# jsign/go-curdleproofs

Hardware: NVIDIA B200
Metric: whisk_shuffle_proof_roundtrips_per_s (GenerateWhiskShuffleProof + IsValidWhiskShuffleProof, n=128) (higher is better)
Workload: dtype u32 (12x32-bit Montgomery limbs, IMAD.WIDE)

## Files before the change

go-curdleproofs_b200/binding.py:

```python
from __future__ import annotations

import ctypes as C
import os
import re

HERE = os.path.dirname(os.path.abspath(__file__))
HEADER = os.path.join(HERE, "..", "include", "curdle_b200.h")

FP_BYTES = 48
FR_BYTES = 32
G1_AFFINE_BYTES = 96
G1_JAC_BYTES = 144


class CdlError(RuntimeError):
    def __init__(self, code: int, msg: str):
        super().__init__(f"curdle_b200 error {code}: {msg}")
        self.code = code
        self.msg = msg


def lib_path() -> str:
    return os.environ.get("CDL_LIB") or os.path.join(HERE, "libcurdle_b200.so")


def declared_symbols():
    txt = open(HEADER).read()
    txt = re.sub(r"/\*.*?\*/", "", txt, flags=re.S)
    return sorted(set(re.findall(r"\b(cdl_[a-z0-9_]+)\s*\(", txt)))


_LIB = None


def load_library():
    global _LIB
    if _LIB is not None:
        return _LIB
    p = lib_path()
    if not os.path.exists(p):
        raise RuntimeError(
            f"{p} is missing: build it with `python -c 'import __graft_entry__ as g; g.build()'` "
            "(nvcc, sm_100a).  There is no CPU fallback.")
    lib = C.CDLL(p)
    vp, sz, i32, u32p = C.c_void_p, C.c_size_t, C.c_int32, C.POINTER(C.c_uint32)
    lib.cdl_abi_version.restype = C.c_uint32
    lib.cdl_create.argtypes = [C.c_int, C.POINTER(vp)]
    lib.cdl_destroy.argtypes = [vp]
    lib.cdl_destroy.restype = None
    lib.cdl_last_error.argtypes = [vp]
    lib.cdl_last_error.restype = C.c_char_p
    lib.cdl_device_info.argtypes = [vp, C.POINTER(i32), C.POINTER(i32), C.c_char_p, sz]
    lib.cdl_g1_msm.argtypes = [vp, vp, vp, sz, vp]
    lib.cdl_g1_msm_batch.argtypes = [vp, vp, vp, u32p, sz, vp]
    lib.cdl_g1_msm_batch_device.argtypes = [vp, vp, vp, vp, vp, sz, vp, vp, vp]
    lib.cdl_g1_scalar_mul_affine.argtypes = [vp, vp, vp, sz, sz, vp]
    lib.cdl_g1_fold.argtypes = [vp, vp, vp, vp, sz]
    lib.cdl_g1_batch_to_affine.argtypes = [vp, vp, sz, vp]
    lib.cdl_g1_sum_affine.argtypes = [vp, vp, sz, vp]
    lib.cdl_g1_compress.argtypes = [vp, vp, sz, vp]
    lib.cdl_g1_decompress.argtypes = [vp, vp, sz, vp, vp]
    lib.cdl_fp_mul.argtypes = [vp, vp, vp, sz, vp]
    lib.cdl_int_peak.argtypes = [vp, C.c_int, C.c_int, C.POINTER(C.c_double), C.POINTER(C.c_double)]
    lib.cdl_int_peak_cfg.argtypes = [vp, C.c_int, C.c_int, C.c_int, C.c_int, C.POINTER(C.c_double), C.POINTER(C.c_double)]
    u64, i32p = C.c_uint64, C.POINTER(C.c_int32)
    lib.cdl_rand_new.argtypes = [u64, C.POINTER(vp)]
    lib.cdl_rand_free.argtypes = [vp]
    lib.cdl_rand_free.restype = None
    lib.cdl_rand_get_frs.argtypes = [vp, sz, vp]
    lib.cdl_rand_get_g1_affines.argtypes = [vp, vp, sz, vp]
    lib.cdl_rand_generate_permutation.argtypes = [vp, sz, u32p]
    lib.cdl_crs_generate.argtypes = [vp, sz, vp, C.POINTER(vp)]
    lib.cdl_crs_from_points.argtypes = [vp, sz, vp, C.POINTER(vp)]
    lib.cdl_crs_export.argtypes = [vp, vp, vp]
    lib.cdl_crs_ell.argtypes = [vp]
    lib.cdl_crs_ell.restype = sz
    lib.cdl_crs_free.argtypes = [vp]
    lib.cdl_crs_free.restype = None
    lib.cdl_shuffle_permute_commit.argtypes = [vp, vp, vp, vp, u32p, vp, vp, vp, vp, vp, vp]
    lib.cdl_prove.argtypes = [vp, vp, vp, vp, vp, vp, vp, u32p, vp, vp, vp, vp, sz, C.POINTER(sz)]
    lib.cdl_verify.argtypes = [vp, vp, vp, sz, vp, vp, vp, vp, vp, vp, i32p]
    lib.cdl_whisk_generate_shuffle_proof.argtypes = [vp, vp, vp, vp, vp, vp, sz]
    lib.cdl_whisk_is_valid_shuffle_proof.argtypes = [vp, vp, vp, vp, sz, sz, vp, sz, vp, i32p]
    lib.cdl_whisk_generate_shuffle_proof_batch.argtypes = [vp, vp, sz, vp, C.POINTER(vp), vp, vp, sz, i32p]
    lib.cdl_whisk_is_valid_shuffle_proof_batch.argtypes = [vp, vp, sz, vp, vp, vp, sz, C.POINTER(vp), i32p, i32p]
    lib.cdl_whisk_generate_tracker_proof_batch.argtypes = [vp, sz, vp, vp, C.POINTER(vp), vp, i32p]
    lib.cdl_whisk_is_valid_tracker_proof_batch.argtypes = [vp, sz, vp, vp, vp, i32p, i32p]
    lib.cdl_whisk_match_trackers.argtypes = [vp, sz, vp, sz, vp, i32p, i32p]
    lib.cdl_host_selftest.argtypes = [vp, vp, vp, vp]
    lib.cdl_host_selftest_fibers.argtypes = [C.c_uint32, C.c_uint32, vp, C.POINTER(C.c_int32)]
    lib.cdl_engine_stats.argtypes = [vp, vp, vp, vp, vp, C.c_int]
    lib.cdl_engine_busy_ms.argtypes = [vp, C.POINTER(C.c_double)]
    lib.cdl_set_lanes.argtypes = [vp, i32]
    lib.cdl_launch_count.argtypes = [vp]
    lib.cdl_launch_count.restype = u64
    f32p = C.POINTER(C.c_float)
    lib.cdl_dev_alloc.argtypes = [vp, sz, C.POINTER(vp)]
    lib.cdl_dev_free.argtypes = [vp, vp]
    lib.cdl_dev_upload.argtypes = [vp, vp, vp, sz]
    lib.cdl_dev_download.argtypes = [vp, vp, vp, sz]
    lib.cdl_g1_scalar_mul_affine_device.argtypes = [vp, vp, vp, sz, sz, vp]
    lib.cdl_g1_fold_device.argtypes = [vp, vp, vp, vp, sz]
    lib.cdl_g1_msm_device.argtypes = [vp, vp, vp, sz, C.c_uint32, C.c_uint32, i32, vp, f32p]
    lib.cdl_set_msm_window.argtypes = [vp, i32]
    lib.cdl_set_msm_batch_affine.argtypes = [vp, i32]
    lib.cdl_set_fixed_base_min_batch.argtypes = [vp, i32]
    lib.cdl_comm_unique_id.argtypes = [vp]
    lib.cdl_comm_init.argtypes = [vp, vp, i32, i32]
    lib.cdl_comm_destroy.argtypes = [vp]
    lib.cdl_comm_partition.argtypes = [sz, i32, i32, i32, i32p, i32p, i32p, i32p]
    lib.cdl_comm_partition.restype = None
    lib.cdl_g1_msm_sharded_device.argtypes = [vp, vp, vp, sz, vp, f32p]
    lib.cdl_g1_msm_sharded.argtypes = [vp, vp, vp, sz, vp]
    no_status = ("cdl_comm_partition", "cdl_destroy", "cdl_last_error", "cdl_abi_version", "cdl_rand_free", "cdl_crs_free", "cdl_crs_ell",
                 "cdl_launch_count")
    for name in declared_symbols():
        fn = getattr(lib, name)
        if name not in no_status:
            fn.restype = i32
    _LIB = lib
    return lib


class Context:

    def __init__(self, device: int = 0):
        self.lib = load_library()
        h = C.c_void_p()
        rc = self.lib.cdl_create(device, C.byref(h))
        if rc != 0:
            raise CdlError(rc, "cdl_create failed (no CUDA device? this library has no CPU fallback)")
        self.h = h

    def close(self):
        if getattr(self, "h", None):
            self.lib.cdl_destroy(self.h)
            self.h = None

    __del__ = close

    def _chk(self, rc: int):
        if rc != 0:
            raise CdlError(rc, (self.lib.cdl_last_error(self.h) or b"").decode())

    def device_info(self):
        sm, khz = C.c_int32(), C.c_int32()
        name = C.create_string_buffer(128)
        self._chk(self.lib.cdl_device_info(self.h, C.byref(sm), C.byref(khz), name, 128))
        return {"sm_count": sm.value, "clock_khz": khz.value, "name": name.value.decode()}

    def g1_msm(self, points: bytes, scalars: bytes) -> bytes:
        n = len(points) // G1_AFFINE_BYTES
        if len(scalars) != n * FR_BYTES:
            raise CdlError(-3, "len(points) != len(scalars)")
        out = C.create_string_buffer(G1_JAC_BYTES)
        self._chk(self.lib.cdl_g1_msm(self.h, points, scalars, n, out))
        return out.raw

    def g1_msm_batch(self, points: bytes, scalars: bytes, offsets) -> bytes:
        k = len(offsets) - 1
        offs = (C.c_uint32 * (k + 1))(*offsets)
        out = C.create_string_buffer(max(1, k) * G1_AFFINE_BYTES)
        self._chk(self.lib.cdl_g1_msm_batch(self.h, points, scalars, offs, k, out))
        return out.raw[: k * G1_AFFINE_BYTES]

    def g1_scalar_mul_affine(self, points: bytes, scalars: bytes, broadcast: bool) -> bytes:
        n = len(points) // G1_AFFINE_BYTES
        out = C.create_string_buffer(max(1, n) * G1_AFFINE_BYTES)
        self._chk(self.lib.cdl_g1_scalar_mul_affine(self.h, points, scalars, n, 0 if broadcast else 1, out))
        return out.raw[: n * G1_AFFINE_BYTES]

    def g1_fold(self, L: bytes, R: bytes, x: bytes) -> bytes:
        n = len(L) // G1_AFFINE_BYTES
        buf = C.create_string_buffer(L, max(1, len(L)))
        self._chk(self.lib.cdl_g1_fold(self.h, buf, R, x, n))
        return buf.raw[: len(L)]

    def g1_batch_to_affine(self, jac: bytes) -> bytes:
        n = len(jac) // G1_JAC_BYTES
        out = C.create_string_buffer(max(1, n) * G1_AFFINE_BYTES)
        self._chk(self.lib.cdl_g1_batch_to_affine(self.h, jac, n, out))
        return out.raw[: n * G1_AFFINE_BYTES]

    def g1_sum_affine(self, points: bytes) -> bytes:
        n = len(points) // G1_AFFINE_BYTES
        out = C.create_string_buffer(G1_AFFINE_BYTES)
        self._chk(self.lib.cdl_g1_sum_affine(self.h, points, n, out))
        return out.raw

    def g1_compress(self, points: bytes) -> bytes:
        n = len(points) // G1_AFFINE_BYTES
        out = C.create_string_buffer(max(1, n) * 48)
        self._chk(self.lib.cdl_g1_compress(self.h, points, n, out))
        return out.raw[: n * 48]

    def g1_decompress(self, enc: bytes, check: bool = True):
        n = len(enc) // 48
        out = C.create_string_buffer(max(1, n) * G1_AFFINE_BYTES)
        st = C.create_string_buffer(max(1, n))
        rc = self.lib.cdl_g1_decompress(self.h, enc, n, out, st)
        if rc != 0 and (check or rc != -4):
            self._chk(rc)
        return out.raw[: n * G1_AFFINE_BYTES], list(st.raw[:n])

    def fp_mul(self, a: bytes, b: bytes) -> bytes:
        n = len(a) // FP_BYTES
        out = C.create_string_buffer(max(1, n) * FP_BYTES)
        self._chk(self.lib.cdl_fp_mul(self.h, a, b, n, out))
        return out.raw[: n * FP_BYTES]

    def int_peak(self, kind: int, iters: int):
        ops, ms = C.c_double(), C.c_double()
        self._chk(self.lib.cdl_int_peak(self.h, kind, iters, C.byref(ops), C.byref(ms)))
        return ops.value, ms.value


def _ctx_int_peak_cfg(self, kind: int, iters: int, blocks_per_sm: int, tpb: int):
    ops, ms = C.c_double(), C.c_double()
    self._chk(self.lib.cdl_int_peak_cfg(self.h, kind, iters, blocks_per_sm, tpb, C.byref(ops), C.byref(ms)))
    return ops.value, ms.value


class DeviceBuffer:

    def __init__(self, ctx: "Context", nbytes: int):
        self.ctx = ctx
        self.nbytes = nbytes
        p = C.c_void_p()
        ctx._chk(ctx.lib.cdl_dev_alloc(ctx.h, nbytes, C.byref(p)))
        self.ptr = p

    def upload(self, data: bytes, offset: int = 0):
        if offset + len(data) > self.nbytes:
            raise ValueError("upload past the end of the device buffer")
        self.ctx._chk(self.ctx.lib.cdl_dev_upload(self.ctx.h, C.c_void_p(self.ptr.value + offset), data, len(data)))

    def download(self, nbytes: int | None = None, offset: int = 0) -> bytes:
        nbytes = self.nbytes - offset if nbytes is None else nbytes
        out = C.create_string_buffer(max(1, nbytes))
        self.ctx._chk(self.ctx.lib.cdl_dev_download(self.ctx.h, out, C.c_void_p(self.ptr.value + offset), nbytes))
        return out.raw[:nbytes]

    def close(self):
        if getattr(self, "ptr", None) and getattr(self.ctx, "h", None):
            self.ctx.lib.cdl_dev_free(self.ctx.h, self.ptr)
        self.ptr = None

    __del__ = close


def comm_unique_id() -> bytes:
    lib = load_library()
    out = C.create_string_buffer(128)
    rc = lib.cdl_comm_unique_id(out)
    if rc != 0:
        raise CdlError(rc, "cdl_comm_unique_id (NCCL unavailable?)")
    return out.raw


def comm_partition(n: int, world: int, rank: int, window_bits: int = 0):
    lib = load_library()
    a, b, c, d = C.c_int32(), C.c_int32(), C.c_int32(), C.c_int32()
    lib.cdl_comm_partition(n, world, rank, window_bits, C.byref(a), C.byref(b), C.byref(c), C.byref(d))
    return a.value, b.value, c.value, d.value


def _ctx_dev_buffer(self, nbytes: int) -> DeviceBuffer:
    return DeviceBuffer(self, nbytes)


def _ctx_g1_scalar_mul_affine_device(self, d_in: DeviceBuffer, d_s: DeviceBuffer, n: int, broadcast: bool,
                                     d_out: DeviceBuffer):
    self._chk(self.lib.cdl_g1_scalar_mul_affine_device(self.h, d_in.ptr, d_s.ptr, n, 0 if broadcast else 1, d_out.ptr))


def _ctx_g1_msm_batch_device(self, d_pool: "DeviceBuffer", idx, scalars: bytes, offsets, out_slot=None, want_affine=True,
                             want_enc=True):
    k = len(offsets) - 1
    ia = (C.c_uint32 * max(1, len(idx)))(*idx)
    oa = (C.c_uint32 * (k + 1))(*offsets)
    sa = (C.c_uint32 * k)(*out_slot) if out_slot is not None else None
    out = C.create_string_buffer(max(1, k) * G1_AFFINE_BYTES) if want_affine else None
    o48 = C.create_string_buffer(max(1, k) * 48) if want_enc else None
    self._chk(self.lib.cdl_g1_msm_batch_device(self.h, d_pool.ptr, ia, scalars, oa, k, sa, out, o48))
    return (out.raw[:k * G1_AFFINE_BYTES] if out else None), (o48.raw[:k * 48] if o48 else None)


def _ctx_g1_fold_device(self, d_L: DeviceBuffer, d_R: DeviceBuffer, d_x: DeviceBuffer, n: int):
    self._chk(self.lib.cdl_g1_fold_device(self.h, d_L.ptr, d_R.ptr, d_x.ptr, n))


def _ctx_g1_msm_device(self, d_points, d_scalars, n: int, part_index: int = 0, part_count: int = 1,
                       normalize: bool = True, d_out: DeviceBuffer | None = None):
    own = d_out is None
    if own:
        d_out = DeviceBuffer(self, G1_JAC_BYTES)
    ms = C.c_float()
    pp = d_points.ptr if isinstance(d_points, DeviceBuffer) else C.c_void_p(int(d_points))
    ps = d_scalars.ptr if isinstance(d_scalars, DeviceBuffer) else C.c_void_p(int(d_scalars))
    self._chk(self.lib.cdl_g1_msm_device(self.h, pp, ps, n, part_index, part_count, 1 if normalize else 0, d_out.ptr,
                                         C.byref(ms)))
    res = d_out.download(G1_JAC_BYTES)
    if own:
        d_out.close()
    return res, ms.value


def _ctx_set_msm_window(self, bits: int):
    self._chk(self.lib.cdl_set_msm_window(self.h, bits))


def _ctx_set_fixed_base_min_batch(self, instances: int):
    self._chk(self.lib.cdl_set_fixed_base_min_batch(self.h, instances))


def _ctx_set_msm_batch_affine(self, rounds: int):
    self._chk(self.lib.cdl_set_msm_batch_affine(self.h, rounds))


def _ctx_comm_init(self, uid: bytes, rank: int, world: int):
    self._chk(self.lib.cdl_comm_init(self.h, uid, rank, world))


def _ctx_comm_destroy(self):
    self._chk(self.lib.cdl_comm_destroy(self.h))


def _ctx_g1_msm_sharded_device(self, d_points: DeviceBuffer, d_scalars: DeviceBuffer, n: int):
    d_out = DeviceBuffer(self, G1_JAC_BYTES)
    ms = C.c_float()
    self._chk(self.lib.cdl_g1_msm_sharded_device(self.h, d_points.ptr, d_scalars.ptr, n, d_out.ptr, C.byref(ms)))
    res = d_out.download(G1_JAC_BYTES)
    d_out.close()
    return res, ms.value


def _ctx_g1_msm_sharded(self, points: bytes, scalars: bytes) -> bytes:
    n = len(points) // G1_AFFINE_BYTES
    if len(scalars) != n * FR_BYTES:
        raise CdlError(-3, "len(points) != len(scalars)")
    out = C.create_string_buffer(G1_JAC_BYTES)
    self._chk(self.lib.cdl_g1_msm_sharded(self.h, points, scalars, n, out))
    return out.raw


class Rand:

    def __init__(self, seed: int):
        self.lib = load_library()
        h = C.c_void_p()
        rc = self.lib.cdl_rand_new(seed, C.byref(h))
        if rc != 0:
            raise CdlError(rc, "cdl_rand_new")
        self.h = h

    def close(self):
        if getattr(self, "h", None):
            self.lib.cdl_rand_free(self.h)
            self.h = None

    __del__ = close

    def get_frs(self, n: int) -> bytes:
        out = C.create_string_buffer(max(1, n) * FR_BYTES)
        rc = self.lib.cdl_rand_get_frs(self.h, n, out)
        if rc != 0:
            raise CdlError(rc, "cdl_rand_get_frs")
        return out.raw[: n * FR_BYTES]

    def get_fr(self) -> bytes:
        return self.get_frs(1)

    def generate_permutation(self, n: int):
        out = (C.c_uint32 * max(1, n))()
        rc = self.lib.cdl_rand_generate_permutation(self.h, n, out)
        if rc != 0:
            raise CdlError(rc, "cdl_rand_generate_permutation")
        return list(out[:n])


class CRS:

    def __init__(self, ctx: "Context", handle):
        self.ctx = ctx
        self.h = handle

    @property
    def ell(self) -> int:
        return self.ctx.lib.cdl_crs_ell(self.h)

    def export(self) -> bytes:
        out = C.create_string_buffer((self.ell + 9) * G1_AFFINE_BYTES)
        self.ctx._chk(self.ctx.lib.cdl_crs_export(self.ctx.h, self.h, out))
        return out.raw

    def close(self):
        if getattr(self, "h", None) and getattr(self.ctx, "h", None):
            self.ctx.lib.cdl_crs_free(self.h)
        self.h = None

    __del__ = close


def _ctx_rand_get_g1_affines(self, rand: Rand, n: int) -> bytes:
    out = C.create_string_buffer(max(1, n) * G1_AFFINE_BYTES)
    self._chk(self.lib.cdl_rand_get_g1_affines(self.h, rand.h, n, out))
    return out.raw[: n * G1_AFFINE_BYTES]


def _ctx_generate_crs(self, ell: int, rand: Rand) -> CRS:
    h = C.c_void_p()
    self._chk(self.lib.cdl_crs_generate(self.h, ell, rand.h, C.byref(h)))
    return CRS(self, h)


def _ctx_crs_from_points(self, ell: int, points: bytes) -> CRS:
    h = C.c_void_p()
    self._chk(self.lib.cdl_crs_from_points(self.h, ell, points, C.byref(h)))
    return CRS(self, h)


def _ctx_shuffle_permute_commit(self, crs: CRS, Rs: bytes, Ss: bytes, perm, k: bytes, rand: Rand):
    ell = crs.ell
    Ts = C.create_string_buffer(ell * G1_AFFINE_BYTES)
    Us = C.create_string_buffer(ell * G1_AFFINE_BYTES)
    M = C.create_string_buffer(G1_JAC_BYTES)
    rs_m = C.create_string_buffer(4 * FR_BYTES)
    p = (C.c_uint32 * ell)(*perm)
    self._chk(self.lib.cdl_shuffle_permute_commit(self.h, crs.h, Rs, Ss, p, k, rand.h, Ts, Us, M, rs_m))
    return Ts.raw, Us.raw, M.raw, rs_m.raw


def _ctx_prove(self, crs: CRS, Rs, Ss, Ts, Us, M, perm, k, rs_m, rand: Rand) -> bytes:
    ell = crs.ell
    cap = 48 * (18 + 10 * 32) + 32 * 7 + 40
    out = C.create_string_buffer(cap)
    n = C.c_size_t()
    p = (C.c_uint32 * ell)(*perm)
    self._chk(self.lib.cdl_prove(self.h, crs.h, Rs, Ss, Ts, Us, M, p, k, rs_m, rand.h, out, cap, C.byref(n)))
    return out.raw[: n.value]


def _ctx_verify(self, crs: CRS, proof: bytes, Rs, Ss, Ts, Us, M, rand: Rand) -> bool:
    ok = C.c_int32()
    self._chk(self.lib.cdl_verify(self.h, crs.h, proof, len(proof), Rs, Ss, Ts, Us, M, rand.h, C.byref(ok)))
    return bool(ok.value)


def _ctx_whisk_generate(self, crs: CRS, pre: bytes, rand: Rand, proof_size: int = 4576):
    ell = crs.ell
    post = C.create_string_buffer(ell * 96)
    proof = C.create_string_buffer(proof_size)
    self._chk(self.lib.cdl_whisk_generate_shuffle_proof(self.h, crs.h, pre, rand.h, post, proof, proof_size))
    return post.raw, proof.raw


def _ctx_whisk_is_valid(self, crs: CRS, pre: bytes, post: bytes, proof: bytes, rand: Rand) -> bool:
    ok = C.c_int32()
    self._chk(self.lib.cdl_whisk_is_valid_shuffle_proof(self.h, crs.h, pre, post, len(pre) // 96, len(post) // 96,
                                                        proof, len(proof), rand.h, C.byref(ok)))
    return bool(ok.value)


def _inbuf(x):
    if isinstance(x, bytes):
        return x
    return (C.c_char * len(x)).from_buffer(x)


def _ctx_whisk_generate_batch(self, crs: CRS, pre, rands, proof_size: int = 4576):
    B = len(rands)
    ell = crs.ell
    post = bytearray(B * ell * 96)
    proofs = bytearray(B * proof_size)
    status = (C.c_int32 * B)()
    rh = (C.c_void_p * B)(*[r.h for r in rands])
    self._chk(self.lib.cdl_whisk_generate_shuffle_proof_batch(self.h, crs.h, B, _inbuf(pre), rh, _inbuf(post), _inbuf(proofs),
                                                              proof_size, status))
    return post, proofs, list(status)


def _ctx_whisk_is_valid_batch(self, crs: CRS, pre, post, proofs, rands, proof_size: int = 4576):
    B = len(rands)
    ok = (C.c_int32 * B)()
    status = (C.c_int32 * B)()
    rh = (C.c_void_p * B)(*[r.h for r in rands])
    self._chk(self.lib.cdl_whisk_is_valid_shuffle_proof_batch(self.h, crs.h, B, _inbuf(pre), _inbuf(post), _inbuf(proofs),
                                                              proof_size, rh, ok, status))
    return list(ok), list(status)


def _ctx_whisk_generate_tracker_proof_batch(self, trackers: bytes, ks: bytes, rands):
    B = len(rands)
    proofs = C.create_string_buffer(B * 128)
    status = (C.c_int32 * B)()
    rh = (C.c_void_p * B)(*[r.h for r in rands])
    self._chk(self.lib.cdl_whisk_generate_tracker_proof_batch(self.h, B, trackers, ks, rh, proofs, status))
    return proofs.raw, list(status)


def _ctx_whisk_is_valid_tracker_proof_batch(self, trackers: bytes, k_comms: bytes, proofs: bytes):
    B = len(trackers) // 96
    ok = (C.c_int32 * B)()
    status = (C.c_int32 * B)()
    self._chk(self.lib.cdl_whisk_is_valid_tracker_proof_batch(self.h, B, trackers, k_comms, proofs, ok, status))
    return list(ok), list(status)


def _ctx_whisk_match_trackers(self, trackers: bytes, ks: bytes):
    T = len(trackers) // 96
    V = len(ks) // 32
    owner = (C.c_int32 * max(T, 1))()
    status = (C.c_int32 * max(T, 1))()
    self._chk(self.lib.cdl_whisk_match_trackers(self.h, T, _inbuf(trackers), V, _inbuf(ks), owner, status))
    return list(owner)[:T], list(status)[:T]


def _ctx_engine_stats(self, reset: bool = False):
    n = (C.c_uint64 * 4)()
    ms = (C.c_double * 4)()
    mm = (C.c_double * 4)()
    by = (C.c_double * 4)()
    self._chk(self.lib.cdl_engine_stats(self.h, n, ms, mm, by, 1 if reset else 0))
    names = ("msm_small", "elem_scalar_mul", "decompress", "compress")
    return {names[i]: {"launches": int(n[i]), "ms": ms[i], "modmul": mm[i], "bytes": by[i]} for i in range(4)}


def _ctx_engine_busy_ms(self) -> float:
    v = C.c_double()
    self._chk(self.lib.cdl_engine_busy_ms(self.h, C.byref(v)))
    return v.value


def _ctx_set_lanes(self, lanes: int):
    self._chk(self.lib.cdl_set_lanes(self.h, lanes))


def _ctx_launch_count(self) -> int:
    return int(self.lib.cdl_launch_count(self.h))


Context.int_peak_cfg = _ctx_int_peak_cfg
Context.dev_buffer = _ctx_dev_buffer
Context.g1_scalar_mul_affine_device = _ctx_g1_scalar_mul_affine_device
Context.g1_fold_device = _ctx_g1_fold_device
Context.g1_msm_batch_device = _ctx_g1_msm_batch_device
Context.g1_msm_device = _ctx_g1_msm_device
Context.set_msm_window = _ctx_set_msm_window
Context.set_msm_batch_affine = _ctx_set_msm_batch_affine
Context.set_fixed_base_min_batch = _ctx_set_fixed_base_min_batch
Context.comm_init = _ctx_comm_init
Context.comm_destroy = _ctx_comm_destroy
Context.g1_msm_sharded_device = _ctx_g1_msm_sharded_device
Context.g1_msm_sharded = _ctx_g1_msm_sharded
Context.rand_get_g1_affines = _ctx_rand_get_g1_affines
Context.generate_crs = _ctx_generate_crs
Context.crs_from_points = _ctx_crs_from_points
Context.shuffle_permute_commit = _ctx_shuffle_permute_commit
Context.prove = _ctx_prove
Context.verify = _ctx_verify
Context.whisk_generate_shuffle_proof = _ctx_whisk_generate
Context.whisk_is_valid_shuffle_proof = _ctx_whisk_is_valid
Context.whisk_generate_shuffle_proof_batch = _ctx_whisk_generate_batch
Context.whisk_is_valid_shuffle_proof_batch = _ctx_whisk_is_valid_batch
Context.whisk_generate_tracker_proof_batch = _ctx_whisk_generate_tracker_proof_batch
Context.whisk_is_valid_tracker_proof_batch = _ctx_whisk_is_valid_tracker_proof_batch
Context.whisk_match_trackers = _ctx_whisk_match_trackers
Context.launch_count = _ctx_launch_count
Context.engine_busy_ms = _ctx_engine_busy_ms
Context.set_lanes = _ctx_set_lanes
Context.engine_stats = _ctx_engine_stats
```

go-curdleproofs_b200/csrc/capi.cu:

```cuda
#include <cstdarg>
#include <cstdio>
#include <cstring>
#include <cstdlib>
#include <mutex>
#include <string>
#include <vector>

#include "../../include/curdle_b200.h"
#include "context.cuh"
#include "host/engine.hpp"
#include "launch.h"

using namespace cdl;

static_assert(sizeof(Fp) == sizeof(cdl_fp), "fp layout");
static_assert(sizeof(Fr) == sizeof(cdl_fr), "fr layout");
static_assert(sizeof(G1Affine) == sizeof(cdl_g1_affine), "affine layout");
static_assert(sizeof(G1Jac) == sizeof(cdl_g1_jac), "jac layout");

static bool msm_tasks(const uint32_t* offsets, size_t k, std::vector<MsmTask>& tasks) {
  tasks.resize(k);
  for (size_t j = 0; j < k; j++) {
    if (offsets[j + 1] < offsets[j]) return false;
    tasks[j] = MsmTask{offsets[j], offsets[j + 1] - offsets[j], (uint32_t)j, 0};
  }
  return true;
}

extern "C" {

uint32_t cdl_abi_version(void) { return (1u << 16) | 5u; }

int32_t cdl_create(int device, cdl_ctx** out) {
  if (!out) return CDL_ERR_INVALID_ARG;
  *out = nullptr;
  int count = 0;
  cudaError_t e = cudaGetDeviceCount(&count);
  if (e != cudaSuccess || count == 0) return CDL_ERR_NO_DEVICE;
  if (device < 0 || device >= count) return CDL_ERR_INVALID_ARG;
  cdl_ctx* c = new cdl_ctx();
  c->device = device;
  if (cudaSetDevice(device) != cudaSuccess || cudaStreamCreateWithFlags(&c->stream, cudaStreamNonBlocking) != cudaSuccess) {
    delete c;
    return CDL_ERR_CUDA;
  }
  cudaDeviceProp prop;
  cudaGetDeviceProperties(&prop, device);
  c->sm_count = prop.multiProcessorCount;
  c->clock_khz = prop.clockRate;
  c->name = prop.name;
  cudaEventCreate(&c->ev0);
  cudaEventCreate(&c->ev1);
  cudaEventCreate(&c->base_ev);
  cudaEventRecord(c->base_ev, c->stream);
  cudaStreamSynchronize(c->stream);
  msm_small_init();
  if (const char* e = getenv("CDL_MSM_C")) c->msm_c_override = atoi(e);
  if (const char* e = getenv("CDL_LANES")) { int v = atoi(e); if (v >= 1 && v <= 16) c->n_lanes = v; }
  *out = c;
  return CDL_OK;
}

cdl_ctx* cdl_lane_(cdl_ctx* root, size_t i) {
  while (root->lanes.size() <= i) {
    cdl_ctx* l = new cdl_ctx();
    l->device = root->device;
    l->sm_count = root->sm_count;
    l->clock_khz = root->clock_khz;
    l->name = root->name;
    l->parent = root;
    l->n_lanes = 1;
    l->msm_c_override = root->msm_c_override;
    if (cudaStreamCreateWithFlags(&l->stream, cudaStreamNonBlocking) != cudaSuccess) { delete l; return nullptr; }
    cudaEventCreate(&l->ev0);
    cudaEventCreate(&l->ev1);
    root->lanes.push_back(l);
  }
  return root->lanes[i];
}

int32_t cdl_set_lanes(cdl_ctx* c, int32_t lanes) {
  if (!c || lanes < 1 || lanes > 16) return CDL_ERR_INVALID_ARG;
  std::lock_guard<std::mutex> lk(c->mu);
  c->n_lanes = lanes;
  return CDL_OK;
}

void cdl_engine_free_(void* engine);
int32_t cdl_big_msm_host_(cdl_ctx* c, const cdl_g1_affine* points, const cdl_fr* scalars, size_t n, cdl_g1_jac* out);

void cdl_destroy(cdl_ctx* c) {
  if (!c) return;
  cudaSetDevice(c->device);
  cdl_comm_destroy(c);
  for (cdl_ctx* l : c->lanes) cdl_destroy(l);
  c->lanes.clear();
  if (c->engine) cdl_engine_free_(c->engine);
  c->free_all();
  cudaEventDestroy(c->ev0);
  cudaEventDestroy(c->ev1);
  if (c->base_ev) cudaEventDestroy(c->base_ev);
  if (c->ev_sync) cudaEventDestroy(c->ev_sync);
  cudaStreamDestroy(c->stream);
  delete c;
}

const char* cdl_last_error(cdl_ctx* c) { return c ? c->err.c_str() : "null context"; }

int32_t cdl_device_info(cdl_ctx* c, int32_t* sm_count, int32_t* clock_khz, char* name, size_t cap) {
  if (!c) return CDL_ERR_INVALID_ARG;
  if (sm_count) *sm_count = c->sm_count;
  if (clock_khz) *clock_khz = c->clock_khz;
  if (name && cap) { strncpy(name, c->name.c_str(), cap - 1); name[cap - 1] = 0; }
  return CDL_OK;
}

int32_t cdl_g1_msm_batch(cdl_ctx* c, const cdl_g1_affine* points, const cdl_fr* scalars,
                         const uint32_t* offsets, size_t k, cdl_g1_affine* out) {
  if (!c || !offsets || !out || (k && offsets[k] && (!points || !scalars))) return CDL_ERR_INVALID_ARG;
  if (k == 0) return CDL_OK;
  std::lock_guard<std::mutex> lk(c->mu);
  const size_t total = offsets[k];
  cdlh::MsmStage st;
  if (!msm_tasks(offsets, k, st.tasks)) return c->fail(CDL_ERR_INVALID_ARG, "msm_batch: offsets not monotone");
  if (k + total >= (1u << 30))
    return c->fail(CDL_ERR_INVALID_ARG, "msm_batch: %zu MSMs of %zu terms exceed the 2^30-point pool", k, total);
  CDL_CUDA(c, cudaSetDevice(c->device));
  c->spin_wait = true;
  cdlh::Engine* E = cdlh::engine_of(c);
  st.idx.resize(total);
  for (size_t t = 0; t < total; t++) st.idx[t] = (uint32_t)(k + t);
  st.sc.assign(reinterpret_cast<const cdlh::Fr*>(scalars), reinterpret_cast<const cdlh::Fr*>(scalars) + total);
  int32_t rc;
  if ((rc = E->ensure_pool(k + total)) || (rc = E->upload_points((uint32_t)k, points, total)) || (rc = E->run_msm(st)))
    return rc;
  return E->download_points(0, out, k);
}

int32_t cdl_g1_msm_batch_device(cdl_ctx* c, cdl_g1_affine* d_pool, const uint32_t* idx, const cdl_fr* scalars,
                                const uint32_t* offsets, size_t k, const uint32_t* out_slot, cdl_g1_affine* out,
                                uint8_t* out48) {
  if (!c || !d_pool || !offsets || (k && offsets[k] && (!idx || !scalars))) return CDL_ERR_INVALID_ARG;
  if (k == 0) return CDL_OK;
  std::lock_guard<std::mutex> lk(c->mu);
  const size_t total = offsets[k];
  cdlh::MsmStage st;
  if (!msm_tasks(offsets, k, st.tasks)) return c->fail(CDL_ERR_INVALID_ARG, "msm_batch_device: offsets not monotone");
  for (size_t t = 0; t < total; t++)
    if (idx[t] & 0x40000000u) return c->fail(CDL_ERR_INVALID_ARG, "msm_batch_device: pool index of term %zu exceeds 2^30 - 1", t);
  CDL_CUDA(c, cudaSetDevice(c->device));
  c->spin_wait = true;
  cdlh::Engine* E = cdlh::engine_of(c);
  st.idx.assign(idx, idx + total);
  st.sc.assign(reinterpret_cast<const cdlh::Fr*>(scalars), reinterpret_cast<const cdlh::Fr*>(scalars) + total);
  int32_t rc;
  if ((rc = E->ensure_pool(k)) || (rc = E->run_msm(st, nullptr, reinterpret_cast<const G1Affine*>(d_pool)))) return rc;
  if (out48) memcpy(out48, st.out48.data(), k * 48);
  if (out_slot) {
    for (size_t j = 0; j < k; j++)
      CDL_CUDA(c, cudaMemcpyAsync(reinterpret_cast<G1Affine*>(d_pool) + out_slot[j], E->d_pool() + j, sizeof(G1Affine),
                                  cudaMemcpyDeviceToDevice, c->stream));
  }
  if (out) return E->download_points(0, out, k);
  CDL_CUDA(c, c->sync_stream());
  return CDL_OK;
}

int32_t cdl_g1_msm(cdl_ctx* c, const cdl_g1_affine* points, const cdl_fr* scalars, size_t n, cdl_g1_jac* out) {
  if (!c || !out || (n && (!points || !scalars))) return CDL_ERR_INVALID_ARG;
  if (n > kBigMsmThreshold) {
    std::lock_guard<std::mutex> lk(c->mu);
    CDL_CUDA(c, cudaSetDevice(c->device));
    return cdl_big_msm_host_(c, points, scalars, n, out);
  }
  uint32_t offs[2] = {0, (uint32_t)n};
  cdl_g1_affine a;
  int32_t rc = cdl_g1_msm_batch(c, points, scalars, offs, 1, &a);
  if (rc != CDL_OK) return rc;
  cdlh::affine_to_jac(out, a);
  return CDL_OK;
}

int32_t cdl_g1_sum_affine(cdl_ctx* c, const cdl_g1_affine* in, size_t n, cdl_g1_affine* out) {
  if (!c || !out || (n && !in)) return CDL_ERR_INVALID_ARG;
// ... 150 lines not shown
```

go-curdleproofs_b200/csrc/capi_protocol.cu:

```cuda
#include <cstring>
#include <memory>
#include <algorithm>
#include <functional>
#include <mutex>
#include <thread>
#include <vector>

#include "host/engine.hpp"

using cdlh::affine_to_jac;
using cdlh::Engine;
using cdlh::engine_of;
using cdlh::Fr;
using cdlh::Layout;

static_assert(sizeof(Fr) == sizeof(cdl_fr), "host fr layout");

extern "C" cdl_ctx* cdl_lane_(cdl_ctx* root, size_t i);

namespace {

const uint32_t kGenX[12] = {0xfd530c16u, 0x5cb38790u, 0x9976fff5u, 0x7817fc67u, 0x143ba1c1u, 0x154f95c7u,
                            0xf3d0e747u, 0xf0ae6acdu, 0x21dbf440u, 0xedce6eccu, 0x9e0bfb75u, 0x12017741u};
const uint32_t kGenY[12] = {0x0ce72271u, 0xbaac93d5u, 0x7918fd8eu, 0x8c22631au, 0x570725ceu, 0xdd595f13u,
// ... 142 lines not shown
      if (modmul) modmul[i] += E->stats.modmul[i];
      if (bytes) bytes[i] += E->stats.bytes[i];
    }
    if (reset) { E->stats = Engine::Stats(); E->intervals.clear(); }
  });
  return CDL_OK;
}

int32_t cdl_engine_busy_ms(cdl_ctx* c, double* busy_ms) {
  if (!c || !busy_ms) return CDL_ERR_INVALID_ARG;
  std::lock_guard<std::mutex> lk(c->mu);
  std::vector<std::pair<float, float>> iv;
  for_each_engine(c, [&](Engine* E) { iv.insert(iv.end(), E->intervals.begin(), E->intervals.end()); });
  std::sort(iv.begin(), iv.end());
  double busy = 0, cur_lo = 0, cur_hi = -1;
  for (auto& p : iv) {
    if (cur_hi < 0 || p.first > cur_hi) {
      if (cur_hi >= 0) busy += cur_hi - cur_lo;
      cur_lo = p.first;
      cur_hi = p.second;
    } else if (p.second > cur_hi) {
      cur_hi = p.second;
    }
  }
  if (cur_hi >= 0) busy += cur_hi - cur_lo;
  *busy_ms = busy;
  return CDL_OK;
}

int32_t cdl_host_selftest(uint8_t* out32, const cdl_fr* a, const cdl_fr* b, cdl_fr* fr_out) {
  if (!out32 || !a || !b || !fr_out) return CDL_ERR_INVALID_ARG;
  cdlh::Transcript t("test protocol");
  t.append_message("some label", reinterpret_cast<const uint8_t*>("some data"), 9);
  t.challenge_bytes("challenge", out32, 32);
  Fr x, y;
  memcpy(&x, a, 32);
  memcpy(&y, b, 32);
  Fr t1 = cdlh::fr_sub(cdlh::fr_add(cdlh::fr_mul(x, y), x), y);
  Fr r = cdlh::fr_mul(cdlh::fr_inv(t1), cdlh::fr_pow_u64(x, 5));
  memcpy(fr_out, &r, 32);
  std::vector<Fr> bi = cdlh::fr_batch_inv({x, t1, cdlh::FR_ZERO, y, t1});
  if (!cdlh::fr_eq(bi[1], cdlh::fr_inv(t1)) || !cdlh::fr_eq(bi[4], bi[1]) || !cdlh::fr_is_zero(bi[2]) ||
      !cdlh::fr_eq(bi[0], cdlh::fr_inv(x)) || !cdlh::fr_eq(bi[3], cdlh::fr_inv(y)))
    return CDL_ERR_INTERNAL;
  if (!cdlh::fr_is_zero(t1) && !cdlh::fr_eq(cdlh::fr_mul(t1, cdlh::fr_inv(t1)), cdlh::FR_ONE)) return CDL_ERR_INTERNAL;
  return CDL_OK;
}

int32_t cdl_host_selftest_fibers(uint32_t n, uint32_t rounds, uint8_t* digest32, int32_t* used_x8) {
  if (!digest32 || !used_x8 || n == 0 || n > (1u << 16)) return CDL_ERR_INVALID_ARG;
  auto work = [&](size_t i, uint8_t* out) {
    cdlh::Transcript t("curdleproofs");
    cdlh::Rand rnd(1000 + i);
    uint8_t msg[200];
    for (uint32_t r = 0; r < rounds; r++) {
      size_t len = 1 + (i * 7 + r * 13) % sizeof msg;
      for (size_t k = 0; k < len; k++) msg[k] = (uint8_t)(i + 31 * r + k);
      t.append_message("selftest_msg", msg, len);
      Fr c = t.challenge("selftest_challenge");
      Fr x = rnd.get_fr();
      t.append_scalar("selftest_rand", x);
      cdlh::fr_to_bytes_be(out + 32 * r, cdlh::fr_add(c, x));
    }
    t.challenge_bytes("selftest_final", out + 32 * rounds, 32);
  };
  const size_t per = (size_t)rounds * 32 + 32;
  std::vector<uint8_t> plain(n * per), fib(n * per);
  for (size_t i = 0; i < n; i++) work(i, plain.data() + i * per);
  *used_x8 = cdlh::fibers_available() ? 1 : 0;
  cdlh::ThreadPool pool(3);
  std::function<void(size_t)> fn([&](size_t i) { work(i, fib.data() + i * per); });
  pool.parallel_for((n + 7) / 8, std::function<void(size_t)>([&](size_t g) {
    cdlh::run_fiber_group(fn, 8 * g, n - 8 * g < 8 ? n - 8 * g : 8);
  }));
  cdlh::Shake256 h;
  h.absorb(fib.data(), fib.size());
  h.read(digest32, 32);
  return plain == fib ? CDL_OK : CDL_ERR_INTERNAL;
}

int32_t cdl_rand_new(uint64_t seed, cdl_rand** out) {
  if (!out) return CDL_ERR_INVALID_ARG;
  *out = new cdl_rand(seed);
  return CDL_OK;
}
void cdl_rand_free(cdl_rand* r) { delete r; }
int32_t cdl_rand_get_frs(cdl_rand* r, size_t n, cdl_fr* out) {
  if (!r || (n && !out)) return CDL_ERR_INVALID_ARG;
  r->r.get_frs(reinterpret_cast<Fr*>(out), n);
  return CDL_OK;
}
int32_t cdl_rand_generate_permutation(cdl_rand* r, size_t n, uint32_t* out) {
  if (!r || (n && !out)) return CDL_ERR_INVALID_ARG;
  std::vector<uint32_t> p = r->r.generate_permutation(n);
  memcpy(out, p.data(), n * 4);
  return CDL_OK;
}
int32_t cdl_rand_get_g1_affines(cdl_ctx* c, cdl_rand* r, size_t n, cdl_g1_affine* out) {
  if (!c || !r || (n && !out)) return CDL_ERR_INVALID_ARG;
  std::lock_guard<std::mutex> lk(c->mu);
  CDL_CUDA(c, cudaSetDevice(c->device));
  Engine* E = engine_of(c);
  int32_t rc;
  if ((rc = E->ensure_pool(n + 1)) || (rc = put_generator(E, 0)) || (rc = rand_points_to_pool(E, r, 0, 1, n))) return rc;
  return E->download_points(1, out, n);
}

int32_t cdl_crs_generate(cdl_ctx* c, size_t ell, cdl_rand* r, cdl_crs** out) {
  if (!c || !r || !out || ell == 0 || ell > (1u << 24)) return CDL_ERR_INVALID_ARG;
  std::lock_guard<std::mutex> lk(c->mu);
  CDL_CUDA(c, cudaSetDevice(c->device));
  Engine* E = engine_of(c);
  Layout L((uint32_t)ell);
  int32_t rc;
  if ((rc = E->ensure_pool(L.crs_size + 1))) return rc;
  const uint32_t gen = L.crs_size;
  if ((rc = put_generator(E, gen))) return rc;
  if ((rc = rand_points_to_pool(E, r, gen, L.Gs, ell + 7))) return rc;
  cdlh::MsmStage st;
  st.idx.resize(ell + 4);
  st.sc.assign(ell + 4, cdlh::FR_ONE);
  for (uint32_t i = 0; i < ell + 4; i++) st.idx[i] = i;
  st.tasks.push_back(cdl::MsmTask{0, (uint32_t)ell, L.Gsum, 0});
  st.tasks.push_back(cdl::MsmTask{(uint32_t)ell, 4, L.Hsum, 0});
  if ((rc = E->run_msm(st))) return rc;
  return crs_finish(c, E, L, out);
}

int32_t cdl_crs_from_points(cdl_ctx* c, size_t ell, const cdl_g1_affine* points, cdl_crs** out) {
  if (!c || !points || !out || ell == 0 || ell > (1u << 24)) return CDL_ERR_INVALID_ARG;
  std::lock_guard<std::mutex> lk(c->mu);
  CDL_CUDA(c, cudaSetDevice(c->device));
  Engine* E = engine_of(c);
  Layout L((uint32_t)ell);
  int32_t rc;
  if ((rc = E->ensure_pool(L.crs_size + 1)) || (rc = E->upload_points(0, points, ell + 9))) return rc;
  return crs_finish(c, E, L, out);
}

int32_t cdl_crs_export(cdl_ctx* c, const cdl_crs* crs, cdl_g1_affine* points) {
  if (!c || !crs || !points) return CDL_ERR_INVALID_ARG;
  std::lock_guard<std::mutex> lk(c->mu);
  CDL_CUDA(c, cudaSetDevice(c->device));
  CDL_CUDA(c, cudaMemcpy(points, crs->d_points, (size_t)(crs->ell + 9) * sizeof(cdl::G1Affine), cudaMemcpyDeviceToHost));
  return CDL_OK;
}

size_t cdl_crs_ell(const cdl_crs* crs) { return crs ? crs->ell : 0; }

int32_t cdl_set_fixed_base_min_batch(cdl_ctx* c, int32_t instances) {
  if (!c || instances < -1) return CDL_ERR_INVALID_ARG;
  std::lock_guard<std::mutex> lk(c->mu);
  c->root()->fixed_min_batch = instances;
  return CDL_OK;
}

void cdl_crs_free(cdl_crs* crs) {
  if (!crs) return;
  if (crs->d_points) { cudaSetDevice(crs->ctx->device); cudaFree(crs->d_points); }
  if (crs->d_fixed) { cudaSetDevice(crs->ctx->device); cudaFree(crs->d_fixed); }
  delete crs;
}

int32_t cdl_shuffle_permute_commit(cdl_ctx* c, const cdl_crs* crs, const cdl_g1_affine* Rs, const cdl_g1_affine* Ss,
                                   const uint32_t* perm, const cdl_fr* k, cdl_rand* r, cdl_g1_affine* Ts,
                                   cdl_g1_affine* Us, cdl_g1_jac* M, cdl_fr* rs_m) {
  if (!c || !crs || !Rs || !Ss || !perm || !k || !r || !Ts || !Us || !M || !rs_m) return CDL_ERR_INVALID_ARG;
  std::lock_guard<std::mutex> lk(c->mu);
  Engine* E;
  Layout L(1);
  int32_t rc = begin_call(c, crs, 1, &E, &L);
  if (rc) return rc;
  const uint32_t ell = L.ell, base = L.base(0);
  for (uint32_t i = 0; i < ell; i++)
    if (perm[i] >= ell) return c->fail(CDL_ERR_INVALID_ARG, "permutation entry out of range");
  if ((rc = E->upload_points(base + L.Rs, Rs, ell)) || (rc = E->upload_points(base + L.Ss, Ss, ell))) return rc;
  std::vector<std::vector<uint32_t>> perms(1, std::vector<uint32_t>(perm, perm + ell));
  std::vector<Fr> ks(1);
  memcpy(&ks[0], k, 32);
  std::vector<cdl_rand*> rands(1, r);
  std::vector<std::vector<Fr>> rsm;
  if ((rc = E->shuffle_permute_commit(L, 1, perms, ks, rands, rsm))) return rc;
  cdl_g1_affine m_aff;
  if ((rc = E->download_points(base + L.Ts, Ts, ell)) || (rc = E->download_points(base + L.Us, Us, ell)) ||
      (rc = E->download_points(base + L.M, &m_aff, 1)))
    return rc;
  affine_to_jac(M, m_aff);
  memcpy(rs_m, rsm[0].data(), 4 * 32);
  return CDL_OK;
}

int32_t cdl_prove(cdl_ctx* c, const cdl_crs* crs, const cdl_g1_affine* Rs, const cdl_g1_affine* Ss,
                  const cdl_g1_affine* Ts, const cdl_g1_affine* Us, const cdl_g1_jac* M, const uint32_t* perm,
                  const cdl_fr* k, const cdl_fr* rs_m, cdl_rand* r, uint8_t* proof, size_t proof_cap,
                  size_t* proof_len) {
  if (!c || !crs || !Rs || !Ss || !Ts || !Us || !M || !perm || !k || !rs_m || !r || !proof || !proof_len)
    return CDL_ERR_INVALID_ARG;
  std::lock_guard<std::mutex> lk(c->mu);
  Engine* E;
  Layout L(1);
  int32_t rc = begin_call(c, crs, 1, &E, &L);
  if (rc) return rc;
  const uint32_t ell = L.ell, base = L.base(0);
  for (uint32_t i = 0; i < ell; i++)
    if (perm[i] >= ell) return c->fail(CDL_ERR_INVALID_ARG, "permutation entry out of range");
  if ((rc = E->upload_points(base + L.Rs, Rs, ell)) || (rc = E->upload_points(base + L.Ss, Ss, ell)) ||
      (rc = E->upload_points(base + L.Ts, Ts, ell)) || (rc = E->upload_points(base + L.Us, Us, ell)) ||
      (rc = E->upload_jac(base + L.M, M, 1)))
    return rc;
  std::vector<std::vector<uint32_t>> perms(1, std::vector<uint32_t>(perm, perm + ell));
  std::vector<Fr> ks(1);
  memcpy(&ks[0], k, 32);
  std::vector<std::vector<Fr>> rsm(1, std::vector<Fr>(4));
  memcpy(rsm[0].data(), rs_m, 4 * 32);
  std::vector<cdl_rand*> rands(1, r);
  std::vector<std::vector<uint8_t>> proofs;
  std::vector<int32_t> status;
  std::vector<std::string> errs;
  std::vector<uint8_t> inst_enc;
  if ((rc = E->prove(L, 1, crs, perms, ks, rsm, rands, proofs, status, errs, inst_enc, false))) return rc;
  if (status[0] != CDL_OK) return c->fail(status[0], "%s", errs[0].c_str());
  *proof_len = proofs[0].size();
  if (proofs[0].size() > proof_cap) return c->fail(CDL_ERR_INVALID_ARG, "proof buffer too small: need %zu bytes", proofs[0].size());
  memcpy(proof, proofs[0].data(), proofs[0].size());
  return CDL_OK;
}

}

namespace {

int32_t load_proofs(Engine* E, const Layout& L, uint32_t B, const uint8_t* const* proof_ptr, const size_t* proof_len,
                    bool with_m, const uint8_t* const* m_enc, const std::vector<const uint8_t*>& inst_enc,
                    bool decode_instance, std::vector<Engine::ParsedProof>& pp) {
  const uint32_t ell = L.ell;
  pp.assign(B, Engine::ParsedProof());
  std::vector<uint8_t> enc;
  std::vector<uint32_t> dst;
  std::vector<uint32_t> owner;
  for (uint32_t b = 0; b < B; b++) {
    Engine::ParsedProof& q = pp[b];
    q.inst_enc = inst_enc[b];
    cdlh::WireProof w;
    size_t used = 0;
    std::string e = cdlh::parse_wire_proof(proof_ptr[b], proof_len[b], with_m, w, &used);
    if (!e.empty()) { q.err = "decoding proof: " + e; continue; }
    q.sc.resize(7);
    bool sc_ok = true;
    for (int i = 0; i < 7; i++) sc_ok = sc_ok && cdlh::fr_from_bytes_be_canonical(q.sc[i], w.scalars[i]);
    if (!sc_ok) { q.err = "decoding proof: scalar is not canonical"; continue; }
    memcpy(q.lens, w.lens, sizeof q.lens);
    if (w.points.size() + (with_m ? 0 : 1) > 19 + 10 * 32) { q.err = "decoding proof: too many points"; continue; }
    const uint32_t base = L.base(b);
    uint32_t slot = base + L.PP;
    if (!with_m) {
      q.pt.push_back(base + L.M);
      q.enc.push_back(m_enc[b]);
    }
    for (const uint8_t* p : w.points) {
      q.pt.push_back(slot);
      q.enc.push_back(p);
      enc.insert(enc.end(), p, p + 48);
      dst.push_back(slot++);
      owner.push_back(b);
    }
    if (decode_instance) {
      enc.insert(enc.end(), inst_enc[b], inst_enc[b] + (size_t)4 * ell * 48);
      for (uint32_t i = 0; i < 4 * ell; i++) { dst.push_back(base + L.Rs + i); owner.push_back(b); }
    }
    q.ok = true;
  }
  std::vector<uint8_t> st;
  int32_t rc = E->decompress(enc.data(), dst, st);
  if (rc) return rc;
  for (size_t i = 0; i < st.size(); i++)
    if (st[i] && pp[owner[i]].ok) {
      pp[owner[i]].ok = false;
      pp[owner[i]].err = "decoding point: rejected encoding (reason " + std::to_string((int)st[i]) + ")";
    }
  return CDL_OK;
}

}

extern "C" {

int32_t cdl_verify(cdl_ctx* c, const cdl_crs* crs, const uint8_t* proof, size_t proof_len,
                   const cdl_g1_affine* Rs, const cdl_g1_affine* Ss, const cdl_g1_affine* Ts,
                   const cdl_g1_affine* Us, const cdl_g1_jac* M, cdl_rand* r, int32_t* ok) {
  if (!c || !crs || !proof || !Rs || !Ss || !Ts || !Us || !M || !r || !ok) return CDL_ERR_INVALID_ARG;
  *ok = 0;
  std::lock_guard<std::mutex> lk(c->mu);
  Engine* E;
  Layout L(1);
  int32_t rc = begin_call(c, crs, 1, &E, &L);
  if (rc) return rc;
  const uint32_t ell = L.ell, base = L.base(0);
  if ((rc = E->upload_points(base + L.Rs, Rs, ell)) || (rc = E->upload_points(base + L.Ss, Ss, ell)) ||
      (rc = E->upload_points(base + L.Ts, Ts, ell)) || (rc = E->upload_points(base + L.Us, Us, ell)) ||
      (rc = E->upload_jac(base + L.M, M, 1)))
    return rc;
  std::vector<uint32_t> src(4 * ell + 1);
  for (uint32_t i = 0; i < 4 * ell; i++) src[i] = base + L.Rs + i;
  src[4 * ell] = base + L.M;
  std::vector<uint8_t> inst;
  if ((rc = E->compress(src, inst))) return rc;
// ... 272 lines not shown
```

go-curdleproofs_b200/csrc/context.cuh:

```cuda
#pragma once
#include <cuda_runtime.h>
#include <cstdarg>
#include <cstdio>
#include <mutex>
#include <string>
#include <vector>

#include "../../include/curdle_b200.h"

struct cdl_ctx {
  int device = 0;
  int sm_count = 0;
  int clock_khz = 0;
  std::string name;
  cudaStream_t stream = nullptr;
  cudaEvent_t ev0 = nullptr, ev1 = nullptr;
  cudaEvent_t ev_sync = nullptr;
  bool spin_wait = false;
  cudaError_t sync_stream() {
    if (spin_wait) return cudaStreamSynchronize(stream);
    if (!ev_sync && cudaEventCreateWithFlags(&ev_sync, cudaEventBlockingSync | cudaEventDisableTiming) != cudaSuccess)
      return cudaStreamSynchronize(stream);
    cudaError_t e = cudaEventRecord(ev_sync, stream);
    if (e != cudaSuccess) return e;
    return cudaEventSynchronize(ev_sync);
  }
  std::mutex mu;
  std::string err;
  void* engine = nullptr;
  void* nccl_comm = nullptr;
  int comm_rank = 0, comm_world = 1;
  int msm_c_override = 0;
  int fixed_min_batch = -1;
  int msm_ba_override = -1;
  cdl_ctx* parent = nullptr;
  std::vector<cdl_ctx*> lanes;
  int n_lanes = 4;
  cudaEvent_t base_ev = nullptr;
  cdl_ctx* root() { return parent ? parent : this; }
  static constexpr int kSlots = 8;
  void* slot[kSlots] = {};
  size_t cap[kSlots] = {};

  void* buf(int i, size_t bytes) {
    if (bytes == 0) bytes = 16;
    if (cap[i] >= bytes) return slot[i];
    if (slot[i]) { cudaStreamSynchronize(stream); cudaFree(slot[i]); slot[i] = nullptr; cap[i] = 0; }
    size_t want = bytes + bytes / 2;
    if (cudaMalloc(&slot[i], want) != cudaSuccess) { slot[i] = nullptr; return nullptr; }
    cap[i] = want;
    return slot[i];
  }
  void free_all() {
    for (int i = 0; i < kSlots; i++) if (slot[i]) { cudaFree(slot[i]); slot[i] = nullptr; cap[i] = 0; }
  }
  int32_t fail(int32_t code, const char* fmt, ...) {
    char tmp[512];
    va_list ap;
    va_start(ap, fmt);
    vsnprintf(tmp, sizeof tmp, fmt, ap);
    va_end(ap);
    err = tmp;
    return code;
  }
};

#define CDL_CUDA(ctx, call)                                                                   \
  do {                                                                                        \
    cudaError_t e__ = (call);                                                                 \
    if (e__ != cudaSuccess)                                                                   \
      return (ctx)->fail(CDL_ERR_CUDA, "%s failed: %s (%s:%d)", #call, cudaGetErrorString(e__), \
                         __FILE__, __LINE__);                                                 \
  } while (0)
```

go-curdleproofs_b200/csrc/engine.cu:

```cuda
#include "host/engine.hpp"

#include <algorithm>
#include <array>
#include <chrono>
#include <cstdio>
#include <cstdlib>
#include <cstring>

using cdl::ElemOp;
using cdl::G1Affine;
using cdl::MsmTask;

namespace cdlh {

static const uint8_t kInfEnc[48] = {0xc0};

Layout::Layout(uint32_t ell_) {
  ell = ell_;
  n = ell + kBlinders;
  m = 0;
  while ((1u << m) < n) m++;
  Gs = 0; Hs = ell; H = ell + 4; Gt = ell + 5; Gu = ell + 6; Gsum = ell + 7; Hsum = ell + 8; INF = ell + 9;
  crs_size = ell + 10;
  uint32_t o = 0;
  Rs = o; o += ell;
  Ss = o; o += ell;
  Ts = o; o += ell;
  Us = o; o += ell;
  M = o++; A = o++; B = o++;
  scratch = o; o += kScratch;
  G = o; o += n;
  Gp = o; o += n;
  Gm = o; o += n;
  Tp = o; o += n;
  Up = o; o += n;
  PP = o; o += 19 + 10 * 32;
  inst_size = o;
}

Engine::Engine(cdl_ctx* ctx)
    : ctx_(ctx),
      pool_(host_threads(ctx->parent != nullptr)) {}

unsigned Engine::host_threads(bool lane) {
  unsigned hw = std::max(1u, std::thread::hardware_concurrency());
  if (const char* e = getenv("CDL_HOST_THREADS")) {
    int v = atoi(e);
    if (v >= 1) hw = std::min(hw, (unsigned)v);
  }
  return lane ? std::max(2u, std::min(32u, hw / 2)) : std::max(1u, std::min(64u, hw));
}

double Engine::now() {
  return std::chrono::duration<double>(std::chrono::steady_clock::now().time_since_epoch()).count();
}

Engine::~Engine() {
  if (getenv("CDL_PROFILE"))
    fprintf(stderr, "[cdl profile] engine %p (lane %d): total %.1f ms = parallel host %.1f + gpu stages %.1f (staging copies %.1f) + serial host %.1f\n",
            (void*)this, ctx_->parent ? 1 : 0, prof.total * 1e3, prof.par * 1e3, prof.gpu * 1e3, prof.copy * 1e3,
            (prof.total - prof.par - prof.gpu) * 1e3);
  cudaSetDevice(ctx_->device);
  if (d_pool_) cudaFree(d_pool_);
  if (d_win_) cudaFree(d_win_);
  if (d_match_) cudaFree(d_match_);
  for (Staging* s : {&s_idx_, &s_sc_, &s_task_, &s_out_, &s_ops_, &s_enc_, &s_st_, &s_jac_, &s_sub_, &s_t2_, &s_cr_, &s_vs_, &s_as_, &s_fsub_}) {
    if (s->h) cudaFreeHost(s->h);
    if (s->d) cudaFree(s->d);
  }
}

double Engine::msm_algorithmic_modmul(uint64_t N) {
  if (N == 0) return 0;
  double best = 1e300;
  for (int c = 1; c <= 24; c++) {
    double W = (double)((256 + c - 1) / c);
    double v = 6.0 * N * W + 28.0 * (double)(1ull << (c - 1)) * W + 9.0 * c * (W - 1) + 14.0 * W;
    if (v < best) best = v;
  }
  return best;
}

void Engine::tick() { cudaEventRecord(ctx_->ev0, ctx_->stream); }
void Engine::tock(int cls, double modmul, double bytes) {
  cudaEventRecord(ctx_->ev1, ctx_->stream);
  pending_cls_ = cls;
  stats.n[cls]++;
  stats.modmul[cls] += modmul;
  stats.bytes[cls] += bytes;
  launches++;
}
void Engine::finish_timing() {
  if (pending_cls_ < 0) return;
  float ms = 0;
  if (cudaEventElapsedTime(&ms, ctx_->ev0, ctx_->ev1) == cudaSuccess) stats.ms[pending_cls_] += ms;
  float t0 = 0;
  if (cudaEventElapsedTime(&t0, ctx_->root()->base_ev, ctx_->ev0) == cudaSuccess && intervals.size() < (1u << 22))
    intervals.emplace_back(t0, t0 + ms);
  pending_cls_ = -1;
}

int32_t Engine::reserve(Staging& s, size_t bytes) {
  if (bytes <= s.cap) return CDL_OK;
  cudaStreamSynchronize(ctx_->stream);
  if (s.h) cudaFreeHost(s.h);
  if (s.d) cudaFree(s.d);
  s.h = s.d = nullptr;
  s.cap = 0;
  size_t want = bytes + bytes / 2 + 256;
  if (cudaMallocHost(&s.h, want) != cudaSuccess || cudaMalloc(&s.d, want) != cudaSuccess)
    return ctx_->fail(CDL_ERR_CUDA, "engine staging allocation of %zu bytes failed", want);
  s.cap = want;
  return CDL_OK;
}

int32_t Engine::ensure_pool(size_t npoints) {
  if (npoints <= pool_cap_) return CDL_OK;
  cudaStreamSynchronize(ctx_->stream);
  if (d_pool_) cudaFree(d_pool_);
  d_pool_ = nullptr;
  pool_cap_ = 0;
  size_t want = npoints + npoints / 4;
  if (cudaMalloc(&d_pool_, want * sizeof(G1Affine)) != cudaSuccess)
    return ctx_->fail(CDL_ERR_CUDA, "point pool allocation of %zu points failed", want);
  pool_cap_ = want;
  return CDL_OK;
}

int32_t Engine::load_crs(const Layout& L, const cdl_crs* crs) {
  CDL_CUDA(ctx_, cudaMemcpyAsync(d_pool_, crs->d_points, (size_t)L.crs_size * sizeof(G1Affine),
                                 cudaMemcpyDeviceToDevice, ctx_->stream));
  return CDL_OK;
}

void Engine::select_fixed(const Layout& L, const cdl_crs* crs, size_t B) {
  fixed_ = cdl::FixedTable();
  static const long min_b = [] {
    const char* e = getenv("CDL_FIXED_BASE_MINB");
    return e ? atol(e) : 64L;
  }();
  const long over = ctx_->root()->fixed_min_batch;
  const long lim = over >= 0 ? over : min_b;
  if (lim <= 0 || (long)B < lim) return;
  std::lock_guard<std::mutex> lk(crs->fixed_mu);
  if (!crs->d_fixed && !crs->fixed_failed) {
    cdl::G1Affine* tab = nullptr;
    if (cudaMalloc(&tab, cdl::fixed_table_bytes(L.crs_size)) != cudaSuccess) {
      cudaGetLastError();
      crs->fixed_failed = true;
      return;
    }
    cdl::launch_fixed_build(crs->d_points, L.crs_size, tab, ctx_->stream);
    if (cudaStreamSynchronize(ctx_->stream) != cudaSuccess) {
      cudaFree(tab);
      crs->fixed_failed = true;
      return;
    }
    crs->d_fixed = tab;
  }
  if (crs->d_fixed) {
    fixed_.tab = crs->d_fixed;
    fixed_.nbase = L.crs_size;
  }
}

int32_t Engine::upload_points(uint32_t dst, const void* host_affine, size_t count) {
  if (!count) return CDL_OK;
  CDL_CUDA(ctx_, cudaMemcpyAsync(d_pool_ + dst, host_affine, count * sizeof(G1Affine), cudaMemcpyHostToDevice, ctx_->stream));
  CDL_CUDA(ctx_, ctx_->sync_stream());
  return CDL_OK;
}

int32_t Engine::upload_jac(uint32_t dst, const void* host_jac, size_t count) {
  if (!count) return CDL_OK;
  int32_t rc = reserve(s_jac_, count * sizeof(cdl::G1Jac));
  if (rc) return rc;
  memcpy(s_jac_.h, host_jac, count * sizeof(cdl::G1Jac));
  CDL_CUDA(ctx_, cudaMemcpyAsync(s_jac_.d, s_jac_.h, count * sizeof(cdl::G1Jac), cudaMemcpyHostToDevice, ctx_->stream));
  tick();
  cdl::launch_jac_to_affine((const cdl::G1Jac*)s_jac_.d, d_pool_ + dst, (int)count, ctx_->stream);
  tock(3, 0, 240.0 * count);
  CDL_CUDA(ctx_, cudaGetLastError());
  CDL_CUDA(ctx_, ctx_->sync_stream());
  finish_timing();
  return CDL_OK;
}

int32_t Engine::download_points(uint32_t src, void* host_affine, size_t count) {
  if (!count) return CDL_OK;
  CDL_CUDA(ctx_, cudaMemcpyAsync(host_affine, d_pool_ + src, count * sizeof(G1Affine), cudaMemcpyDeviceToHost, ctx_->stream));
  CDL_CUDA(ctx_, ctx_->sync_stream());
  return CDL_OK;
}

int32_t Engine::copy_points(uint32_t dst, uint32_t src, size_t count) {
  if (!count) return CDL_OK;
  CDL_CUDA(ctx_, cudaMemcpyAsync(d_pool_ + dst, d_pool_ + src, count * sizeof(G1Affine), cudaMemcpyDeviceToDevice, ctx_->stream));
  return CDL_OK;
}

int32_t Engine::set_infinity(uint32_t dst, size_t count) {
  if (!count) return CDL_OK;
  CDL_CUDA(ctx_, cudaMemsetAsync(d_pool_ + dst, 0, count * sizeof(G1Affine), ctx_->stream));
  return CDL_OK;
}

int32_t Engine::copy_ranges(const std::vector<cdl::CopyRange>& ranges) {
  const size_t n = ranges.size();
  if (!n) return CDL_OK;
  CDL_CUDA(ctx_, ctx_->sync_stream());
  int32_t rc = reserve(s_cr_, n * sizeof(cdl::CopyRange));
  if (rc) return rc;
  memcpy(s_cr_.h, ranges.data(), n * sizeof(cdl::CopyRange));
  CDL_CUDA(ctx_, cudaMemcpyAsync(s_cr_.d, s_cr_.h, n * sizeof(cdl::CopyRange), cudaMemcpyHostToDevice, ctx_->stream));
  cdl::launch_copy_ranges(d_pool_, (const cdl::CopyRange*)s_cr_.d, (int)n, ctx_->stream);
  CDL_CUDA(ctx_, cudaGetLastError());
  launches++;
  return CDL_OK;
}

namespace {
struct ProfScope {
  double& acc;
  double t0;
  explicit ProfScope(double& a) : acc(a), t0(Engine::now()) {}
  ~ProfScope() { acc += Engine::now() - t0; }
};
}

int32_t Engine::compress(const std::vector<uint32_t>& src, std::vector<uint8_t>& out48) {
  ProfScope ps(prof.gpu);
  size_t n = src.size();
  out48.resize(n * 48);
  if (!n) return CDL_OK;
  int32_t rc;
  if ((rc = reserve(s_idx_, n * 4)) || (rc = reserve(s_out_, n * 48))) return rc;
  memcpy(s_idx_.h, src.data(), n * 4);
  CDL_CUDA(ctx_, cudaMemcpyAsync(s_idx_.d, s_idx_.h, n * 4, cudaMemcpyHostToDevice, ctx_->stream));
  tick();
  cdl::launch_compress_idx(d_pool_, (const uint32_t*)s_idx_.d, (uint8_t*)s_out_.d, (int)n, ctx_->stream);
  tock(3, 3.0 * n, 148.0 * n);
  CDL_CUDA(ctx_, cudaGetLastError());
  CDL_CUDA(ctx_, cudaMemcpyAsync(s_out_.h, s_out_.d, n * 48, cudaMemcpyDeviceToHost, ctx_->stream));
  CDL_CUDA(ctx_, ctx_->sync_stream());
  finish_timing();
  memcpy(out48.data(), s_out_.h, n * 48);
  return CDL_OK;
}

int32_t Engine::decompress(const uint8_t* enc48, const std::vector<uint32_t>& dst, std::vector<uint8_t>& status) {
  ProfScope ps(prof.gpu);
  size_t n = dst.size();
  status.assign(n, 0);
  if (!n) return CDL_OK;
  int32_t rc;
  if ((rc = reserve(s_idx_, n * 4)) || (rc = reserve(s_enc_, n * 48)) || (rc = reserve(s_st_, n))) return rc;
  memcpy(s_idx_.h, dst.data(), n * 4);
  memcpy(s_enc_.h, enc48, n * 48);
  CDL_CUDA(ctx_, cudaMemcpyAsync(s_idx_.d, s_idx_.h, n * 4, cudaMemcpyHostToDevice, ctx_->stream));
  CDL_CUDA(ctx_, cudaMemcpyAsync(s_enc_.d, s_enc_.h, n * 48, cudaMemcpyHostToDevice, ctx_->stream));
  tick();
  cdl::launch_decompress_idx((const uint8_t*)s_enc_.d, d_pool_, (const uint32_t*)s_idx_.d, (uint8_t*)s_st_.d, (int)n, ctx_->stream);
  tock(2, (480.0 + 3193.0) * n, 148.0 * n);
  CDL_CUDA(ctx_, cudaGetLastError());
  CDL_CUDA(ctx_, cudaMemcpyAsync(s_st_.h, s_st_.d, n, cudaMemcpyDeviceToHost, ctx_->stream));
  CDL_CUDA(ctx_, ctx_->sync_stream());
  finish_timing();
  memcpy(status.data(), s_st_.h, n);
  return CDL_OK;
}

static constexpr uint32_t kFixedMinTerms = 16;

int32_t Engine::run_msm(MsmStage& st, const std::function<int32_t(cdl::Fr* d_scalars)>& before,
                        const G1Affine* points) {
  ProfScope ps(prof.gpu);
  size_t nt = st.tasks.size(), nterm = st.idx.size();
  st.out48.resize(nt * 48);
  if (!nt) return CDL_OK;
  if (!points) points = d_pool_;
  size_t max_terms = 0;
  for (auto& t : st.tasks) max_terms = std::max<size_t>(max_terms, t.term_cnt);
  int32_t rc;
  if ((rc = reserve(s_idx_, (nterm + 1) * 4)) || (rc = reserve(s_sc_, (nterm + 1) * 32)) ||
      (rc = reserve(s_task_, nt * sizeof(MsmTask))) || (rc = reserve(s_out_, nt * 48)))
    return rc;
  static_assert(cdl::kMsmSplitTerms <= cdl::kMsmMaxTerms, "small-MSM tasks must fit the kernel's staging");
  const bool throughput = (int)nt >= cdl::kMsmSplitThreshold || max_terms > cdl::kMsmSplitTerms;
  std::vector<uint32_t> fixed_tasks;
  {
    ProfScope pc(prof.copy);
    memcpy(s_idx_.h, st.idx.data(), nterm * 4);
    memcpy(s_sc_.h, st.sc.data(), nterm * 32);
    memcpy(s_task_.h, st.tasks.data(), nt * sizeof(MsmTask));
    if (throughput && fixed_.tab) {
      uint32_t* idx = (uint32_t*)s_idx_.h;
      for (size_t j = 0; j < nt; j++) {
        const MsmTask& t = st.tasks[j];
        uint32_t cnt = 0;
        for (uint32_t k = 0; k < t.term_cnt; k++) cnt += (idx[t.term_off + k] & 0x7fffffffu) < fixed_.nbase;
        if (cnt < kFixedMinTerms) continue;
        for (uint32_t k = 0; k < t.term_cnt; k++)
          if ((idx[t.term_off + k] & 0x7fffffffu) < fixed_.nbase) idx[t.term_off + k] |= cdl::kMsmIdxFixed;
        fixed_tasks.push_back((uint32_t)j);
      }
    }
  }
  CDL_CUDA(ctx_, cudaMemcpyAsync(s_idx_.d, s_idx_.h, nterm * 4, cudaMemcpyHostToDevice, ctx_->stream));
  CDL_CUDA(ctx_, cudaMemcpyAsync(s_sc_.d, s_sc_.h, nterm * 32, cudaMemcpyHostToDevice, ctx_->stream));
  CDL_CUDA(ctx_, cudaMemcpyAsync(s_task_.d, s_task_.h, nt * sizeof(MsmTask), cudaMemcpyHostToDevice, ctx_->stream));
  if (before) {
    int32_t brc = before((cdl::Fr*)s_sc_.d);
    if (brc) return brc;
  }
  double alg = 0;
  for (size_t j = 0; j < st.tasks.size(); j++)
    alg += msm_algorithmic_modmul(st.tasks[j].term_cnt - (st.extra.size() == st.tasks.size() ? st.extra[j] : 0));
  if (throughput) {
    std::vector<cdl::MsmSub> subs;
    std::vector<cdl::MsmTask2> tasks2;
    cdl::msm_build_subs(st.tasks.data(), nt, cdl::msm_tp_pick_chunk(nterm, ctx_->sm_count), subs, tasks2);
    if ((rc = reserve(s_sub_, subs.size() * sizeof(cdl::MsmSub))) || (rc = reserve(s_t2_, tasks2.size() * sizeof(cdl::MsmTask2))))
      return rc;
    size_t wb = cdl::msm_tp_scratch_bytes(nterm, subs.size(), nt);
    if (wb > win_cap_) {
      cudaStreamSynchronize(ctx_->stream);
      if (d_win_) cudaFree(d_win_);
      d_win_ = nullptr;
      win_cap_ = 0;
      if (cudaMalloc(&d_win_, wb + wb / 4) != cudaSuccess) return ctx_->fail(CDL_ERR_CUDA, "MSM scratch allocation failed");
      win_cap_ = wb + wb / 4;
    }
    std::vector<uint32_t> fsubs;
    for (uint32_t j : fixed_tasks)
      for (uint32_t c = 0; c < tasks2[j].sub_cnt; c++) fsubs.push_back(tasks2[j].sub_off + c);
    if (!fsubs.empty()) {
      if ((rc = reserve(s_fsub_, fsubs.size() * 4))) return rc;
      memcpy(s_fsub_.h, fsubs.data(), fsubs.size() * 4);
      CDL_CUDA(ctx_, cudaMemcpyAsync(s_fsub_.d, s_fsub_.h, fsubs.size() * 4, cudaMemcpyHostToDevice, ctx_->stream));
    }
    memcpy(s_sub_.h, subs.data(), subs.size() * sizeof(cdl::MsmSub));
    memcpy(s_t2_.h, tasks2.data(), tasks2.size() * sizeof(cdl::MsmTask2));
    CDL_CUDA(ctx_, cudaMemcpyAsync(s_sub_.d, s_sub_.h, subs.size() * sizeof(cdl::MsmSub), cudaMemcpyHostToDevice, ctx_->stream));
    CDL_CUDA(ctx_, cudaMemcpyAsync(s_t2_.d, s_t2_.h, tasks2.size() * sizeof(cdl::MsmTask2), cudaMemcpyHostToDevice, ctx_->stream));
    tick();
    cdl::launch_msm_tp(points, (const uint32_t*)s_idx_.d, (const cdl::Fr*)s_sc_.d, (int)nterm, (const cdl::MsmSub*)s_sub_.d,
                       (int)subs.size(), (const cdl::MsmTask2*)s_t2_.d, (int)nt, d_pool_, (uint8_t*)s_out_.d, d_win_,
                       ctx_->stream, fixed_, fsubs.empty() ? nullptr : (const uint32_t*)s_fsub_.d, (int)fsubs.size());
    tock(0, alg, 128.0 * nterm);
    launches += fsubs.empty() ? 3 : 4;
  } else {
    tick();
    cdl::launch_msm_small(points, (const uint32_t*)s_idx_.d, (const cdl::Fr*)s_sc_.d, (const MsmTask*)s_task_.d, (int)nt,
                          max_terms, d_pool_, (uint8_t*)s_out_.d, ctx_->stream);
    tock(0, alg, 128.0 * nterm);
  }
  CDL_CUDA(ctx_, cudaGetLastError());
  CDL_CUDA(ctx_, cudaMemcpyAsync(s_out_.h, s_out_.d, nt * 48, cudaMemcpyDeviceToHost, ctx_->stream));
  CDL_CUDA(ctx_, ctx_->sync_stream());
  finish_timing();
  memcpy(st.out48.data(), s_out_.h, nt * 48);
  return CDL_OK;
}

int32_t Engine::run_elem(const std::vector<ElemOp>& ops, const std::vector<Fr>& sc) {
  ProfScope ps(prof.gpu);
  size_t n = ops.size();
  if (!n) return CDL_OK;
  int32_t rc;
  if ((rc = reserve(s_ops_, n * sizeof(ElemOp))) || (rc = reserve(s_sc_, sc.size() * 32))) return rc;
  memcpy(s_ops_.h, ops.data(), n * sizeof(ElemOp));
  memcpy(s_sc_.h, sc.data(), sc.size() * 32);
  CDL_CUDA(ctx_, cudaMemcpyAsync(s_ops_.d, s_ops_.h, n * sizeof(ElemOp), cudaMemcpyHostToDevice, ctx_->stream));
  CDL_CUDA(ctx_, cudaMemcpyAsync(s_sc_.d, s_sc_.h, sc.size() * 32, cudaMemcpyHostToDevice, ctx_->stream));
  tick();
  cdl::launch_elem_ops(d_pool_, (const ElemOp*)s_ops_.d, (const cdl::Fr*)s_sc_.d, (int)n, ctx_->stream, fixed_);
  tock(1, 3193.0 * n, 288.0 * n);
  CDL_CUDA(ctx_, cudaGetLastError());
  CDL_CUDA(ctx_, ctx_->sync_stream());
  finish_timing();
  return CDL_OK;
}

namespace {

struct StageBuilder {
  MsmStage& st;
  uint32_t B, terms_per, tasks_per;
  StageBuilder(MsmStage& s, uint32_t B_, uint32_t terms, uint32_t tasks) : st(s), B(B_), terms_per(terms), tasks_per(tasks) {
    st.idx.assign((size_t)B * terms, 0);
    st.sc.assign((size_t)B * terms, FR_ZERO);
    st.tasks.assign((size_t)B * tasks, MsmTask{0, 0, 0, 0});
    st.extra.assign((size_t)B * tasks, 0);
  }
  MsmSlice slice(uint32_t b) {
    MsmSlice s;
    s.idx = st.idx.data() + (size_t)b * terms_per;
    s.sc = st.sc.data() + (size_t)b * terms_per;
    s.tasks = st.tasks.data() + (size_t)b * tasks_per;
    s.extra = st.extra.data() + (size_t)b * tasks_per;
    s.term_base = b * terms_per;
    return s;
  }
  const uint8_t* out(uint32_t b, uint32_t task) const { return st.out48.data() + ((size_t)b * tasks_per + task) * 48; }
};

inline bool is_inf_enc(const uint8_t* e) { return memcmp(e, kInfEnc, 48) == 0; }

constexpr uint32_t kStep3SplitBatch = 8;

}

int32_t Engine::shuffle_permute_commit(const Layout& L, uint32_t B, const std::vector<std::vector<uint32_t>>& perms,
                                       const std::vector<Fr>& ks, std::vector<cdl_rand*>& rands,
                                       std::vector<std::vector<Fr>>& rs_m) {
  ProfScope ptot(prof.total);
  const uint32_t ell = L.ell;
  std::vector<ElemOp> ops((size_t)B * 2 * ell);
  std::vector<Fr> sc(B);
  for (uint32_t b = 0; b < B; b++) {
    uint32_t base = L.base(b);
    sc[b] = ks[b];
    for (uint32_t i = 0; i < ell; i++) {
      ops[(size_t)b * 2 * ell + i] = ElemOp{base + L.Rs + perms[b][i], cdl::kNoPoint, base + L.Ts + i, b};
      ops[(size_t)b * 2 * ell + ell + i] = ElemOp{base + L.Ss + perms[b][i], cdl::kNoPoint, base + L.Us + i, b};
    }
  }
  int32_t rc = run_elem(ops, sc);
  if (rc) return rc;
  MsmStage st;
  StageBuilder sb(st, B, ell + kBlinders, 1);
  rs_m.assign(B, std::vector<Fr>(kBlinders));
  std::vector<Fr> small(ell);
  for (uint32_t j = 0; j < ell; j++) small[j] = fr_from_u64(j);
  for (uint32_t b = 0; b < B; b++) {
    rands[b]->r.get_frs(rs_m[b].data(), kBlinders);
    MsmSlice s = sb.slice(b);
    s.begin(L.base(b) + L.M);
    for (uint32_t i = 0; i < ell; i++) s.term(L.Gs + i, small[perms[b][i]]);
    for (uint32_t j = 0; j < kBlinders; j++) s.term(L.Hs + j, rs_m[b][j]);
    s.end();
  }
  return run_msm(st);
}

namespace {

struct ProveState {
  Transcript tr{"curdleproofs"};
  bool failed = false;
  std::string err;
  std::vector<Fr> as, perm_as, rs_a, bs, rs_b, cs, ds, r_cs, x, r;
  Fr alpha, beta, p, r_p, z, r_t, r_u, r_a, r_b, r_k, z_k, z_t, z_u;
  Fr beta_ipa;
  uint8_t A[48], T1[48], T2[48], U1[48], U2[48], R[48], S[48], Bp[48], C[48], B_c[48], B_d[48];
  uint8_t A1[48], A2[48], B1[48], B2[48], B_a[48], B_t[48], B_u[48];
  std::vector<uint8_t> L_C, R_C, L_D, R_D, L_A, L_T, L_U, R_A, R_T, R_U;
  Fr c0, d0, x0;
  void fail(const std::string& e) { if (!failed) { failed = true; err = e; } }
};

bool generate_ipa_blinders(Rand& rand, const std::vector<Fr>& cs, const std::vector<Fr>& ds, std::vector<Fr>& rs,
                           std::vector<Fr>& zs, std::string& err) {
  size_t n = cs.size();
  rs.resize(n);
  zs.resize(n - 2);
// ... 654 lines not shown
```

go-curdleproofs_b200/csrc/engine_verify.cu:

```cuda
#include <algorithm>
#include <array>
#include <cstring>

#include "host/engine.hpp"

using cdl::MsmTask;

namespace cdlh {

namespace {

const uint8_t kInfEncV[48] = {0xc0};

struct VState {
  Transcript tr{"curdleproofs"};
  bool failed = false;
  std::string err;
  bool late_failed = false;
  std::string late_err;
  std::vector<Fr> as;
  Fr sp_alpha, sp_beta, p, gp_alpha, gp_beta, gp_beta_inv, z;
  Rand snapshot{0};
  bool have_snapshot = false;
  void fail(const std::string& e) { if (!failed) { failed = true; err = e; } }
};

struct Wire {
  uint32_t M = 0, A = 1, T1 = 2, T2 = 3, U1 = 4, U2 = 5, R = 6, S = 7, B = 8, C = 9, B_c = 10, B_d = 11;
  uint32_t L_C, R_C, L_D, R_D, A1, A2, B1, B2, B_a, B_t, B_u, L_A, L_T, L_U, R_A, R_T, R_U, total;
  explicit Wire(const uint32_t* lens) {
    uint32_t o = 12;
    L_C = o; o += lens[0];
    R_C = o; o += lens[1];
    L_D = o; o += lens[2];
    R_D = o; o += lens[3];
    A1 = o++; A2 = o++; B1 = o++; B2 = o++;
    B_a = o++; B_t = o++; B_u = o++;
    L_A = o; o += lens[4];
    L_T = o; o += lens[5];
    L_U = o; o += lens[6];
    R_A = o; o += lens[7];
    R_T = o; o += lens[8];
    R_U = o; o += lens[9];
    total = o;
  }
};

}

int32_t Engine::verify(const Layout& L, uint32_t B, const cdl_crs* crs, std::vector<ParsedProof>& pp,
                       std::vector<cdl_rand*>& rands, std::vector<int32_t>& verdict, std::vector<int32_t>& status,
                       std::vector<std::string>& errs) {
  struct Tot { double& a; double t0; ~Tot() { a += Engine::now() - t0; } } ptot{prof.total, now()};
  const uint32_t ell = L.ell, n = L.n;
  int32_t rc;
  verdict.assign(B, 0);
  status.assign(B, CDL_OK);
  errs.assign(B, "");
  std::vector<std::unique_ptr<VState>> S(B);
  for (auto& s : S) s.reset(new VState());
  const uint8_t* H_enc = crs->enc.data() + 48 * (size_t)L.H;
  MsmStage st;

  for (uint32_t b = 0; b < B; b++)
    if (!pp[b].ok) S[b]->fail(pp[b].err);

  std::vector<std::array<uint8_t, 48>> Aprime(B), Denc(B);

  par(B, [&](size_t b) {
    VState& s = *S[b];
    if (s.failed) return;
    const ParsedProof& q = pp[b];
    Wire w(q.lens);
    const uint8_t* ie = q.inst_enc;
    if (memcmp(ie + (size_t)2 * ell * 48, kInfEncV, 48) == 0) { s.fail("randomizer is zero"); return; }
    s.tr.append_points("curdleproofs_step1", ie, 4 * ell);
    s.tr.append_points("curdleproofs_step1", q.enc[w.M], 1);
    s.as.resize(ell);
    for (uint32_t i = 0; i < ell; i++) s.as[i] = s.tr.challenge("curdleproofs_vec_a");
    s.tr.append_points("same_perm_step1", q.enc[w.A], 1);
    s.tr.append_points("same_perm_step1", q.enc[w.M], 1);
    s.tr.append_scalars("same_perm_step1", s.as.data(), ell);
    s.sp_alpha = s.tr.challenge("same_perm_alpha");
    s.sp_beta = s.tr.challenge("same_perm_beta");
    s.p = FR_ONE;
    Fr i_alpha = FR_ZERO;
    for (uint32_t i = 0; i < ell; i++) {
      s.p = fr_mul(s.p, fr_add(fr_add(i_alpha, s.sp_beta), s.as[i]));
      i_alpha = fr_add(i_alpha, s.sp_alpha);
    }
    s.tr.append_points("gprod_step1", q.enc[w.B], 1);
    s.tr.append_scalar("gprod_step1", s.p);
    s.gp_alpha = s.tr.challenge("gprod_alpha");
    s.tr.append_points("gprod_step2", q.enc[w.C], 1);
    s.tr.append_scalar("gprod_step2", q.sc[0]);
    s.gp_beta = s.tr.challenge("gprod_beta");
    if (fr_is_zero(s.gp_beta)) { s.fail("beta is zero"); return; }
    s.gp_beta_inv = fr_inv(s.gp_beta);
  });

  {
    st.clear();
    std::vector<int> slot(B, -1);
    for (uint32_t b = 0; b < B; b++) {
      VState& s = *S[b];
      if (s.failed) continue;
      const ParsedProof& q = pp[b];
      Wire w(q.lens);
      slot[b] = (int)st.tasks.size();
      st.tasks.push_back(MsmTask{(uint32_t)st.idx.size(), 3, L.base(b) + L.scratch + 1, 0});
      st.idx.push_back(q.pt[w.B]); st.sc.push_back(FR_ONE);
      st.idx.push_back(L.Gsum); st.sc.push_back(fr_neg(s.gp_beta_inv));
      st.idx.push_back(L.Hsum); st.sc.push_back(s.gp_alpha);
      st.tasks.push_back(MsmTask{(uint32_t)st.idx.size(), 3, L.base(b) + L.scratch, 0});
      st.idx.push_back(q.pt[w.A]); st.sc.push_back(FR_ONE);
      st.idx.push_back(q.pt[w.T1]); st.sc.push_back(FR_ONE);
      st.idx.push_back(q.pt[w.U1]); st.sc.push_back(FR_ONE);
    }
    if ((rc = run_msm(st))) return rc;
    for (uint32_t b = 0; b < B; b++)
      if (slot[b] >= 0) {
        memcpy(Denc[b].data(), st.out48.data() + 48 * (size_t)slot[b], 48);
        memcpy(Aprime[b].data(), st.out48.data() + 48 * ((size_t)slot[b] + 1), 48);
      }
  }

  std::vector<std::vector<uint32_t>> t_idx(B);
  std::vector<std::vector<Fr>> t_sc(B);
  std::vector<std::vector<uint32_t>> t_cnt(B);
  std::vector<uint8_t> have_big(B, 0);
  static const bool device_scalars = [] {
    const char* e = getenv("CDL_VERIFY_SCALARS");
    return !(e && e[0] == 'h');
  }();
  const bool dev_sc = device_scalars && L.m <= (uint32_t)cdl::kVsMaxM;
  std::vector<cdl::VsParams> vsp(dev_sc ? B : 0);
  std::vector<uint32_t> merged_at(B, 0);
  par(B, [&](size_t b) {
    VState& s = *S[b];
    if (s.failed) return;
    const ParsedProof& q = pp[b];
    Wire w(q.lens);
    Rand& rand = rands[b]->r;
    const uint32_t base = L.base((uint32_t)b);
    const Fr &Rp = q.sc[0], &c0 = q.sc[1], &d0 = q.sc[2], &Zk = q.sc[3], &Zt = q.sc[4], &Zu = q.sc[5], &xf = q.sc[6];
    std::vector<Fr> sGs(ell, FR_ZERO), sTs(ell, FR_ZERO), sUs(ell, FR_ZERO), sRs(ell, FR_ZERO), sSs(ell, FR_ZERO);
    Fr sHs[4] = {FR_ZERO, FR_ZERO, FR_ZERO, FR_ZERO}, sH = FR_ZERO, sGt = FR_ZERO, sGu = FR_ZERO;
    std::vector<uint32_t>& idx = t_idx[b];
    std::vector<Fr>& sc = t_sc[b];
    auto neg_term = [&](uint32_t point, const Fr& coeff) { idx.push_back(point); sc.push_back(fr_neg(coeff)); };

    Fr a1 = rand.get_fr();
    const Fr a1b = fr_mul(a1, s.sp_beta);
    if (!dev_sc)
      for (uint32_t i = 0; i < ell; i++) sGs[i] = a1b;
    neg_term(q.pt[w.B], a1);
    neg_term(q.pt[w.A], fr_neg(a1));
    neg_term(q.pt[w.M], fr_neg(fr_mul(a1, s.sp_alpha)));

    std::vector<Fr> us(dev_sc ? 0 : n);
    if (!dev_sc) {
      Fr t = s.gp_beta_inv;
      for (uint32_t i = 0; i < ell; i++) { us[i] = t; t = fr_mul(t, s.gp_beta_inv); }
      for (uint32_t i = ell; i < n; i++) us[i] = t;
    }
    Fr beta_l = fr_pow_u64(s.gp_beta, ell);
    Fr beta_l1 = fr_mul(beta_l, s.gp_beta);
    s.z = fr_sub(fr_add(fr_mul(s.p, beta_l), fr_mul(Rp, beta_l1)), FR_ONE);
    s.tr.append_points("ipa_step1", q.enc[w.C], 1);
    s.tr.append_points("ipa_step1", Denc[b].data(), 1);
    s.tr.append_scalar("ipa_step1", s.z);
    s.tr.append_points("ipa_step1", q.enc[w.B_c], 1);
    s.tr.append_points("ipa_step1", q.enc[w.B_d], 1);
    Fr ipa_alpha = s.tr.challenge("ipa_alpha");
    Fr ipa_beta = s.tr.challenge("ipa_beta");
    if (n & (n - 1)) { s.fail("ipa n is not a power of two"); return; }
    const uint32_t m = L.m;
    if (q.lens[0] < m || q.lens[1] < m || q.lens[2] < m || q.lens[3] < m) { s.fail("ipa proof has too few rounds"); return; }
    std::vector<Fr> gamma(m);
    for (uint32_t i = 0; i < m; i++) {
      s.tr.append_points("ipa_loop", q.enc[w.L_C + i], 1);
      s.tr.append_points("ipa_loop", q.enc[w.L_D + i], 1);
      s.tr.append_points("ipa_loop", q.enc[w.R_C + i], 1);
      s.tr.append_points("ipa_loop", q.enc[w.R_D + i], 1);
      gamma[i] = s.tr.challenge("ipa_gamma");
    }
    if (q.lens[0] != m || q.lens[1] != m || q.lens[2] != m || q.lens[3] != m) { s.fail("ipa multiexp: length mismatch"); return; }
    std::vector<Fr> gamma_inv = fr_batch_inv(gamma);
    std::vector<Fr> sv(dev_sc ? 0 : n), svp(dev_sc ? 0 : n);
    if (!dev_sc) {
      sv[0] = svp[0] = FR_ONE;
      for (uint32_t j = 0; j < m; j++)
        for (uint32_t i = 0; i < (1u << j); i++) {
          sv[i + (1u << j)] = fr_mul(sv[i], gamma[m - j - 1]);
          svp[i + (1u << j)] = fr_mul(svp[i], gamma_inv[m - j - 1]);
        }
    }
    Fr a2 = rand.get_fr();
    const Fr a2c0 = fr_mul(a2, c0);
    if (!dev_sc) {
      for (uint32_t i = 0; i < ell; i++) sGs[i] = fr_add(sGs[i], fr_mul(a2c0, sv[i]));
      for (uint32_t j = 0; j < 4; j++) sHs[j] = fr_add(sHs[j], fr_mul(a2c0, sv[ell + j]));
    }
    sH = fr_add(sH, fr_mul(a2, fr_mul(fr_mul(ipa_beta, d0), c0)));
    for (uint32_t i = 0; i < m; i++) {
      neg_term(q.pt[w.L_C + i], fr_mul(a2, gamma[i]));
      neg_term(q.pt[w.R_C + i], fr_mul(a2, gamma_inv[i]));
    }
    neg_term(q.pt[w.B_c], a2);
    neg_term(q.pt[w.C], fr_mul(a2, ipa_alpha));
    sH = fr_sub(sH, fr_mul(a2, fr_mul(fr_mul(fr_mul(ipa_alpha, ipa_alpha), s.z), ipa_beta)));
    Fr a3 = rand.get_fr();
    const Fr a3d0 = fr_mul(a3, d0);
    if (!dev_sc) {
      for (uint32_t i = 0; i < ell; i++) sGs[i] = fr_add(sGs[i], fr_mul(a3d0, fr_mul(svp[i], us[i])));
      for (uint32_t j = 0; j < 4; j++) sHs[j] = fr_add(sHs[j], fr_mul(a3d0, fr_mul(svp[ell + j], us[ell + j])));
    }
    for (uint32_t i = 0; i < m; i++) {
      neg_term(q.pt[w.L_D + i], fr_mul(a3, gamma[i]));
      neg_term(q.pt[w.R_D + i], fr_mul(a3, gamma_inv[i]));
    }
    neg_term(q.pt[w.B_d], a3);
    neg_term(base + L.scratch + 1, fr_mul(a3, ipa_alpha));
    s.snapshot = rand;
    s.have_snapshot = true;

    const uint8_t* seq[10] = {q.enc[w.R], q.enc[w.S], q.enc[w.T1], q.enc[w.T2], q.enc[w.U1], q.enc[w.U2],
                              q.enc[w.A1], q.enc[w.A2], q.enc[w.B1], q.enc[w.B2]};
    for (auto e : seq) s.tr.append_points("sameexp_points", e, 1);
    Fr ss_alpha = s.tr.challenge("sameexp_alpha");
    std::vector<uint32_t> small_idx;
    std::vector<Fr> small_sc;
    auto eq_task = [&](std::initializer_list<std::pair<uint32_t, Fr>> terms) {
      for (auto& t : terms) { small_idx.push_back(t.first); small_sc.push_back(t.second); }
      t_cnt[b].push_back((uint32_t)terms.size());
    };
    eq_task({{q.pt[w.A1], FR_ONE}, {q.pt[w.T1], ss_alpha}, {L.Gt, fr_neg(Zt)}});
    eq_task({{q.pt[w.A2], FR_ONE}, {q.pt[w.T2], ss_alpha}, {q.pt[w.R], fr_neg(Zk)}, {L.H, fr_neg(Zt)}});
    eq_task({{q.pt[w.B1], FR_ONE}, {q.pt[w.U1], ss_alpha}, {L.Gu, fr_neg(Zu)}});
    eq_task({{q.pt[w.B2], FR_ONE}, {q.pt[w.U2], ss_alpha}, {q.pt[w.S], fr_neg(Zk)}, {L.H, fr_neg(Zu)}});

    auto late = [&](const char* e) { s.late_failed = true; s.late_err = e; };
    s.tr.append_points("same_msm_step1", Aprime[b].data(), 1);
    s.tr.append_points("same_msm_step1", q.enc[w.T2], 1);
    s.tr.append_points("same_msm_step1", q.enc[w.U2], 1);
    const uint8_t* ie = q.inst_enc;
    s.tr.append_points("same_msm_step1", ie + (size_t)2 * ell * 48, ell);
    s.tr.append_points("same_msm_step1", kInfEncV, 1);
    s.tr.append_points("same_msm_step1", kInfEncV, 1);
    s.tr.append_points("same_msm_step1", H_enc, 1);
    s.tr.append_points("same_msm_step1", kInfEncV, 1);
    s.tr.append_points("same_msm_step1", ie + (size_t)3 * ell * 48, ell);
    s.tr.append_points("same_msm_step1", kInfEncV, 1);
    s.tr.append_points("same_msm_step1", kInfEncV, 1);
    s.tr.append_points("same_msm_step1", kInfEncV, 1);
    s.tr.append_points("same_msm_step1", H_enc, 1);
    s.tr.append_points("same_msm_step1", q.enc[w.B_a], 1);
    s.tr.append_points("same_msm_step1", q.enc[w.B_t], 1);
    s.tr.append_points("same_msm_step1", q.enc[w.B_u], 1);
    Fr sm_alpha = s.tr.challenge("same_msm_alpha");
    const uint32_t lg_n = q.lens[4];
    if (lg_n >= 32) late("recursive steps greater than expected");
    else if (n != (1u << lg_n)) late("must by log2(L_a)");
    else if (q.lens[5] != lg_n || q.lens[6] != lg_n || q.lens[7] != lg_n || q.lens[8] != lg_n || q.lens[9] != lg_n)
      late("same msm proof: inconsistent round counts");
    if (!s.late_failed) {
      std::vector<Fr> ch(lg_n);
      for (uint32_t i = 0; i < lg_n; i++) {
        s.tr.append_points("same_msm_loop", q.enc[w.L_A + i], 1);
        s.tr.append_points("same_msm_loop", q.enc[w.L_T + i], 1);
        s.tr.append_points("same_msm_loop", q.enc[w.L_U + i], 1);
        s.tr.append_points("same_msm_loop", q.enc[w.R_A + i], 1);
        s.tr.append_points("same_msm_loop", q.enc[w.R_T + i], 1);
        s.tr.append_points("same_msm_loop", q.enc[w.R_U + i], 1);
        ch[i] = s.tr.challenge("same_msm_gamma");
      }
      std::vector<Fr> ch_inv = fr_batch_inv(ch);
      std::vector<Fr> xs(dev_sc ? 0 : n);
      if (!dev_sc) {
        xs[0] = xf;
        for (uint32_t j = 0; j < lg_n; j++)
          for (uint32_t i = 0; i < (1u << j); i++) xs[i + (1u << j)] = fr_mul(xs[i], ch[lg_n - 1 - j]);
      }
      Fr a4 = rand.get_fr();
      if (!dev_sc) {
        for (uint32_t i = 0; i < ell; i++) sGs[i] = fr_add(sGs[i], fr_mul(a4, xs[i]));
        sHs[0] = fr_add(sHs[0], fr_mul(a4, xs[ell]));
        sHs[1] = fr_add(sHs[1], fr_mul(a4, xs[ell + 1]));
        sGt = fr_add(sGt, fr_mul(a4, xs[ell + 2]));
        sGu = fr_add(sGu, fr_mul(a4, xs[ell + 3]));
      }
      neg_term(q.pt[w.B_a], a4);
      neg_term(base + L.scratch, fr_mul(a4, sm_alpha));
      for (uint32_t i = 0; i < lg_n; i++) {
        neg_term(q.pt[w.L_A + i], fr_mul(a4, ch[i]));
        neg_term(q.pt[w.R_A + i], fr_mul(a4, ch_inv[i]));
      }
      Fr a5 = rand.get_fr();
      if (!dev_sc) {
        for (uint32_t i = 0; i < ell; i++) sTs[i] = fr_add(sTs[i], fr_mul(a5, xs[i]));
        sH = fr_add(sH, fr_mul(a5, xs[ell + 2]));
      }
      neg_term(q.pt[w.B_t], a5);
      neg_term(q.pt[w.T2], fr_mul(a5, sm_alpha));
      for (uint32_t i = 0; i < lg_n; i++) {
        neg_term(q.pt[w.L_T + i], fr_mul(a5, ch[i]));
        neg_term(q.pt[w.R_T + i], fr_mul(a5, ch_inv[i]));
      }
      Fr a6 = rand.get_fr();
      if (!dev_sc) {
        for (uint32_t i = 0; i < ell; i++) sUs[i] = fr_add(sUs[i], fr_mul(a6, xs[i]));
        sH = fr_add(sH, fr_mul(a6, xs[ell + 3]));
      }
      neg_term(q.pt[w.B_u], a6);
      neg_term(q.pt[w.U2], fr_mul(a6, sm_alpha));
      for (uint32_t i = 0; i < lg_n; i++) {
        neg_term(q.pt[w.L_U + i], fr_mul(a6, ch[i]));
        neg_term(q.pt[w.R_U + i], fr_mul(a6, ch_inv[i]));
      }
      Fr a7 = rand.get_fr();
      if (!dev_sc)
        for (uint32_t i = 0; i < ell; i++) sRs[i] = fr_mul(a7, s.as[i]);
      neg_term(q.pt[w.R], a7);
      Fr a8 = rand.get_fr();
      if (!dev_sc)
        for (uint32_t i = 0; i < ell; i++) sSs[i] = fr_mul(a8, s.as[i]);
      neg_term(q.pt[w.S], a8);
      if (dev_sc) {
        cdl::VsParams& P = vsp[b];
        auto put = [](cdl::Fr& d, const Fr& v) { memcpy(&d, &v, 32); };
        put(P.a1b, a1b); put(P.a2c0, a2c0); put(P.a3d0, a3d0);
        put(P.a4xf, fr_mul(a4, xf)); put(P.a5xf, fr_mul(a5, xf)); put(P.a6xf, fr_mul(a6, xf));
        put(P.a7, a7); put(P.a8, a8); put(P.beta_inv, s.gp_beta_inv); put(P.sH_host, sH);
        for (uint32_t i = 0; i < m; i++) { put(P.gamma[i], gamma[i]); put(P.gamma_inv[i], gamma_inv[i]); put(P.ch[i], ch[i]); }
        P.sc_base = 0;
        P.as_base = (uint32_t)(b * ell);
        P.pad[0] = P.pad[1] = 0;
      }
      merged_at[b] = (uint32_t)idx.size();
      for (uint32_t i = 0; i < ell; i++) { idx.push_back(L.Gs + i); sc.push_back(sGs[i]); }
      for (uint32_t j = 0; j < 4; j++) { idx.push_back(L.Hs + j); sc.push_back(sHs[j]); }
      idx.push_back(L.H); sc.push_back(sH);
      idx.push_back(L.Gt); sc.push_back(sGt);
      idx.push_back(L.Gu); sc.push_back(sGu);
      for (uint32_t i = 0; i < ell; i++) { idx.push_back(base + L.Ts + i); sc.push_back(sTs[i]); }
      for (uint32_t i = 0; i < ell; i++) { idx.push_back(base + L.Us + i); sc.push_back(sUs[i]); }
      for (uint32_t i = 0; i < ell; i++) { idx.push_back(base + L.Rs + i); sc.push_back(sRs[i]); }
      for (uint32_t i = 0; i < ell; i++) { idx.push_back(base + L.Ss + i); sc.push_back(sSs[i]); }
      have_big[b] = 1;
    }
    uint32_t big_terms = have_big[b] ? (uint32_t)idx.size() : 0;
    std::vector<uint32_t> all_idx(small_idx);
    std::vector<Fr> all_sc(small_sc);
    if (have_big[b]) {
      all_idx.insert(all_idx.end(), idx.begin(), idx.end());
      all_sc.insert(all_sc.end(), sc.begin(), sc.end());
      t_cnt[b].push_back(big_terms);
    }
    idx.swap(all_idx);
    sc.swap(all_sc);
  });

  st.clear();
  std::vector<int> first_task(B, -1);
  std::vector<cdl::VsParams> vs_launch;
  vs_launch.reserve(dev_sc ? B : 0);
  for (uint32_t b = 0; b < B; b++) {
    if (S[b]->failed) continue;
    first_task[b] = (int)st.tasks.size();
    uint32_t off = (uint32_t)st.idx.size();
    st.idx.insert(st.idx.end(), t_idx[b].begin(), t_idx[b].end());
    st.sc.insert(st.sc.end(), t_sc[b].begin(), t_sc[b].end());
    if (dev_sc && have_big[b]) {
      uint32_t small_terms = 0;
      for (size_t t = 0; t + 1 < t_cnt[b].size(); t++) small_terms += t_cnt[b][t];
      vsp[b].sc_base = off + small_terms + merged_at[b];
      vs_launch.push_back(vsp[b]);
    }
    uint32_t k = 0;
    for (uint32_t cnt : t_cnt[b]) {
      st.tasks.push_back(MsmTask{off, cnt, L.base(b) + L.scratch + 2 + k, 0});
      off += cnt;
      k++;
    }
  }
  if (dev_sc && !vs_launch.empty()) {
    const size_t np = vs_launch.size();
    if ((rc = reserve(s_vs_, np * sizeof(cdl::VsParams))) || (rc = reserve(s_as_, (size_t)B * ell * 32))) return rc;
    memcpy(s_vs_.h, vs_launch.data(), np * sizeof(cdl::VsParams));
    Fr* as_h = (Fr*)s_as_.h;
    par(B, [&](size_t b) {
      if (have_big[b]) memcpy(as_h + b * ell, S[b]->as.data(), (size_t)ell * 32);
    });
    CDL_CUDA(ctx_, cudaMemcpyAsync(s_vs_.d, s_vs_.h, np * sizeof(cdl::VsParams), cudaMemcpyHostToDevice, ctx_->stream));
    CDL_CUDA(ctx_, cudaMemcpyAsync(s_as_.d, s_as_.h, (size_t)B * ell * 32, cudaMemcpyHostToDevice, ctx_->stream));
    rc = run_msm(st, [&](cdl::Fr* d_sc) -> int32_t {
      cdl::launch_verify_scalars((const cdl::VsParams*)s_vs_.d, (const cdl::Fr*)s_as_.d, d_sc, (uint32_t)np, ell, n, L.m,
                                 ctx_->stream);
      launches++;
      return CDL_OK;
    });
  } else {
    rc = run_msm(st);
  }
  if (rc) return rc;
  for (uint32_t b = 0; b < B; b++) {
    VState& s = *S[b];
    if (s.failed) { status[b] = CDL_ERR_PROTOCOL; errs[b] = s.err; continue; }
    const uint8_t* o = st.out48.data() + 48 * (size_t)first_task[b];
    bool same_scalar_ok = true;
    for (int t = 0; t < 4; t++) same_scalar_ok = same_scalar_ok && memcmp(o + 48 * t, kInfEncV, 48) == 0;
    if (!same_scalar_ok) {
      verdict[b] = 0;
      if (s.have_snapshot) rands[b]->r = s.snapshot;
      continue;
    }
    if (s.late_failed) {
      status[b] = CDL_ERR_PROTOCOL;
      errs[b] = "verifying same multiscalar: " + s.late_err;
      if (s.have_snapshot) rands[b]->r = s.snapshot;
      continue;
    }
    verdict[b] = memcmp(o + 48 * 4, kInfEncV, 48) == 0 ? 1 : 0;
  }
  return CDL_OK;
}

}
```

go-curdleproofs_b200/csrc/host/engine.hpp:

```cpp
#pragma once
#include <cstdint>
#include <functional>
#include <memory>
#include <string>
#include <vector>

#include "../context.cuh"
#include "../launch.h"
#include "fr.hpp"
#include "pool.hpp"
#include "transcript.hpp"

struct cdl_rand {
  cdlh::Rand r;
  explicit cdl_rand(uint64_t seed) : r(seed) {}
};

struct cdl_crs {
  cdl_ctx* ctx = nullptr;
  uint32_t ell = 0;
  cdl::G1Affine* d_points = nullptr;
  std::vector<uint8_t> enc;
  mutable std::mutex fixed_mu;
  mutable cdl::G1Affine* d_fixed = nullptr;
  mutable bool fixed_failed = false;
};

namespace cdlh {

constexpr uint32_t kBlinders = 4;

struct Layout {
  uint32_t ell, n, m;
  uint32_t Gs, Hs, H, Gt, Gu, Gsum, Hsum, INF, crs_size;
  uint32_t Rs, Ss, Ts, Us, M, A, B, scratch, G, Gp, Gm, Tp, Up, PP, inst_size;
  static constexpr uint32_t kScratch = 24;
  explicit Layout(uint32_t ell_);
  uint32_t base(uint32_t b) const { return crs_size + b * inst_size; }
  uint32_t npp() const { return 19 + 10 * m; }
};

struct MsmStage {
  std::vector<uint32_t> idx;
  std::vector<Fr> sc;
  std::vector<cdl::MsmTask> tasks;
  std::vector<uint8_t> out48;
  std::vector<uint32_t> extra;
  void clear() { idx.clear(); sc.clear(); tasks.clear(); extra.clear(); }
};

struct MsmSlice {
  uint32_t* idx;
  Fr* sc;
  cdl::MsmTask* tasks;
  uint32_t* extra = nullptr;
  uint32_t term_base;
  uint32_t nterm = 0, ntask = 0;
  void begin(uint32_t out_idx) {
    tasks[ntask].term_off = term_base + nterm;
    tasks[ntask].term_cnt = 0;
    tasks[ntask].out_idx = out_idx;
    tasks[ntask].pad = 0;
  }
  void term(uint32_t point, const Fr& s) {
    idx[nterm] = point;
    sc[nterm] = s;
    nterm++;
    tasks[ntask].term_cnt++;
  }
  void term_more(uint32_t point, const Fr& s) {
    term(point, s);
    if (extra) extra[ntask]++;
  }
  void end() { ntask++; }
};

class Engine {
 public:
  explicit Engine(cdl_ctx* ctx);
  ~Engine();

  int32_t shuffle_permute_commit(const Layout& L, uint32_t B, const std::vector<std::vector<uint32_t>>& perms,
                                 const std::vector<Fr>& ks, std::vector<cdl_rand*>& rands,
                                 std::vector<std::vector<Fr>>& rs_m);
  int32_t prove(const Layout& L, uint32_t B, const cdl_crs* crs, const std::vector<std::vector<uint32_t>>& perms,
                const std::vector<Fr>& ks, const std::vector<std::vector<Fr>>& rs_m, std::vector<cdl_rand*>& rands,
                std::vector<std::vector<uint8_t>>& proofs, std::vector<int32_t>& status,
                std::vector<std::string>& errs, std::vector<uint8_t>& inst_enc, bool witness_is_ours);
  struct ParsedProof {
    bool ok = false;
    std::string err;
    uint32_t lens[10] = {};
    std::vector<uint32_t> pt;
    std::vector<const uint8_t*> enc;
    std::vector<Fr> sc;
    const uint8_t* inst_enc = nullptr;
  };
  int32_t verify(const Layout& L, uint32_t B, const cdl_crs* crs, std::vector<ParsedProof>& pp,
                 std::vector<cdl_rand*>& rands, std::vector<int32_t>& verdict, std::vector<int32_t>& status,
                 std::vector<std::string>& errs);

  int32_t ensure_pool(size_t npoints);
  int32_t load_crs(const Layout& L, const cdl_crs* crs);
  void select_fixed(const Layout& L, const cdl_crs* crs, size_t B);
  void clear_fixed() { fixed_ = cdl::FixedTable(); }
  int32_t upload_points(uint32_t dst, const void* host_affine, size_t count);
  int32_t upload_jac(uint32_t dst, const void* host_jac, size_t count);
  int32_t download_points(uint32_t src, void* host_affine, size_t count);
  int32_t copy_points(uint32_t dst, uint32_t src, size_t count);
  int32_t set_infinity(uint32_t dst, size_t count);
  int32_t copy_ranges(const std::vector<cdl::CopyRange>& ranges);
  int32_t compress(const std::vector<uint32_t>& src, std::vector<uint8_t>& out48);
  int32_t decompress(const uint8_t* enc48, const std::vector<uint32_t>& dst, std::vector<uint8_t>& status);
  int32_t run_msm(MsmStage& st, const std::function<int32_t(cdl::Fr* d_scalars)>& before = nullptr,
                  const cdl::G1Affine* points = nullptr);
  int32_t run_elem(const std::vector<cdl::ElemOp>& ops, const std::vector<Fr>& sc);
  int32_t match_trackers(uint32_t T, const Fr* ks, uint32_t V, int32_t* owner);

  cdl_ctx* ctx() { return ctx_; }
  cdl::G1Affine* d_pool() { return d_pool_; }
  ThreadPool& threads() { return pool_; }
  uint64_t launches = 0;
  std::vector<std::pair<float, float>> intervals;
  struct Stats {
    uint64_t n[4] = {};
    double ms[4] = {};
    double modmul[4] = {};
    double bytes[4] = {};
  } stats;
  static double msm_algorithmic_modmul(uint64_t terms);
  struct HostProf {
    double par = 0;
    double gpu = 0;
    double copy = 0;
    double total = 0;
  } prof;
  template <class F>
  void par(size_t n, F&& f) {
    double t0 = now();
    std::function<void(size_t)> fn(std::forward<F>(f));
    if (n >= 4 && fibers_available()) {
      const size_t groups = (n + 7) / 8;
      pool_.parallel_for(groups, std::function<void(size_t)>([&](size_t g) {
        run_fiber_group(fn, 8 * g, n - 8 * g < 8 ? n - 8 * g : 8);
      }));
    } else {
      pool_.parallel_for(n, fn);
    }
    prof.par += now() - t0;
  }
  static double now();
  static unsigned host_threads(bool lane);

 private:
  cdl_ctx* ctx_;
  ThreadPool pool_;
  cdl::G1Affine* d_pool_ = nullptr;
  cdl::FixedTable fixed_;
  size_t pool_cap_ = 0;
  void* d_win_ = nullptr;
  size_t win_cap_ = 0;
  void* d_match_ = nullptr;
  size_t match_cap_ = 0;
  bool match_scratch(uint32_t tile);
  struct Staging {
    void* h = nullptr;
    void* d = nullptr;
    size_t cap = 0;
  };
  Staging s_idx_, s_sc_, s_task_, s_out_, s_ops_, s_enc_, s_st_, s_jac_, s_sub_, s_t2_, s_cr_, s_fsub_, s_vs_, s_as_;
  int32_t reserve(Staging& s, size_t bytes);
  void tick();
  void tock(int cls, double modmul, double bytes);
  int pending_cls_ = -1;
  void finish_timing();
};

struct WireProof {
  std::vector<const uint8_t*> points;
  uint32_t lens[10];
  const uint8_t* scalars[7];
};
std::string parse_wire_proof(const uint8_t* buf, size_t len, bool with_m, WireProof& out, size_t* used);

Engine* engine_of(cdl_ctx* c);
void affine_to_jac(cdl_g1_jac* out, const cdl_g1_affine& a);

}
```

go-curdleproofs_b200/csrc/k_msm_big.cu:

```cuda
#define CDL_FP_MUL_CALL 1
#include <cstdlib>
#include "quad.cuh"
#include "batch_affine.cuh"
#include "launch.h"

namespace cdl {

constexpr uint32_t kBigLargeBucket = 2048;
constexpr uint32_t kBigSliceLen = 2048;
constexpr int kBigCtaThreads = 128;

struct BigSliceRec {
  uint32_t first, count;
};
struct BigLargeRec {
  uint32_t bucket, slice_first, slice_count, pad;
};

struct alignas(128) BigPoint {
  Fp x, y;
  uint32_t pad[8];
};

struct BigSrc {
  const BigPoint* tab;
  uint32_t n;
  const uint32_t* entries;
  const G1Affine* direct;
};
template <bool DIRECT>
__device__ __forceinline__ G1Affine big_src_load(const BigSrc& s, uint32_t t) {
  if (DIRECT) return s.direct[t];
  G1Affine q;
  const uint32_t en = s.entries[t];
  const uint32_t pi = en & 0x7fffffffu;
  if (pi >= 2u * s.n) {
    aff_set_inf(q);
    return q;
  }
  q.x = s.tab[pi].x;
  q.y = s.tab[pi].y;
  if (en >> 31) FpM::neg(q.y, q.y);
  return q;
}
template <bool DIRECT>
__device__ __forceinline__ Fp big_src_load_x(const BigSrc& s, uint32_t t) {
  if (DIRECT) return s.direct[t].x;
  const uint32_t pi = s.entries[t] & 0x7fffffffu;
  if (pi >= 2u * s.n) {
    Fp x;
    FpM::set_zero(x);
    return x;
  }
  return s.tab[pi].x;
}

__device__ __forceinline__ uint32_t big_raw_digit(const uint32_t* k6, int w, int c) {
  int bit = w * c;
  int word = bit >> 5, sh = bit & 31;
  uint32_t lo = k6[word], hi = k6[word + 1];
  uint32_t v = __funnelshift_r(lo, hi, sh);
  return v & ((1u << c) - 1u);
}

__global__ void __launch_bounds__(256)
k_big_tables(const G1Affine* __restrict__ points, int n, BigPoint* __restrict__ tab) {
  int i = blockIdx.x * blockDim.x + threadIdx.x;
  if (i >= n) return;
  const G1Affine p = points[i];
  Fp beta, bx;
  fp_set_beta(beta);
  FpM::mul(bx, p.x, beta);
  tab[i].x = p.x;
  tab[i].y = p.y;
  tab[i + n].x = bx;
  tab[i + n].y = p.y;
}

template <int PASS>
__global__ void __launch_bounds__(256)
k_big_digits(const Fr* __restrict__ scalars, int n, BigMsmDims dm, uint32_t* __restrict__ counters,
             const uint32_t* __restrict__ offsets, uint32_t* __restrict__ entries) {
  const int i = blockIdx.x * blockDim.x + threadIdx.x;
  const bool live = i < n;
  uint32_t k6[2][6];
  bool neg[2] = {false, false};
#pragma unroll
  for (int h = 0; h < 2; h++)
#pragma unroll
    for (int j = 0; j < 6; j++) k6[h][j] = 0;
  if (live) {
    Fr km = scalars[i], k;
    FrM::from_mont(k, km);
    Glv g;
    glv_decompose(g, k.v);
#pragma unroll
    for (int j = 0; j < 4; j++) { k6[0][j] = g.k1[j]; k6[1][j] = g.k2[j]; }
    neg[0] = g.neg1;
    neg[1] = g.neg2;
  }
  const uint32_t lane = threadIdx.x & 31;
#pragma unroll 1
  for (int h = 0; h < 2; h++) {
    uint32_t carry = 0;
    int next_local = dm.wfirst, j = 0;
#pragma unroll 1
    for (int w = 0; w < dm.W; w++) {
      uint32_t t = (w * dm.c < 128 ? big_raw_digit(k6[h], w, dm.c) : 0u) + carry;
      carry = t > (uint32_t)dm.M ? 1u : 0u;
      if (w != next_local) continue;
      int32_t d = carry ? (int32_t)t - (int32_t)(2 * dm.M) : (int32_t)t;
      uint32_t key = 0xffffffffu;
      if (live && d != 0) key = (uint32_t)j * (uint32_t)dm.M + (uint32_t)(d < 0 ? -d : d) - 1u;
      uint32_t peers = __match_any_sync(0xffffffffu, key);
      uint32_t leader = __ffs(peers) - 1;
      uint32_t rank = __popc(peers & ((1u << lane) - 1u));
      uint32_t base = 0;
      if (key != 0xffffffffu && lane == leader) base = atomicAdd(&counters[key], (uint32_t)__popc(peers));
      base = __shfl_sync(0xffffffffu, base, leader);
      if (PASS == 1 && key != 0xffffffffu)
        entries[offsets[key] + base + rank] =
            ((uint32_t)i + (h ? (uint32_t)n : 0u)) | (((d < 0) != neg[h]) ? 0x80000000u : 0u);
      next_local += dm.wstep;
      j++;
    }
  }
}

constexpr int kScanMaxIpt = 16;

__global__ void __launch_bounds__(256)
k_scan_block_sums(const uint32_t* __restrict__ in, uint32_t n, int ipt, uint32_t pad, uint32_t* __restrict__ bsum) {
  __shared__ uint32_t sh[256];
  uint32_t base = (blockIdx.x * 256u + threadIdx.x) * (uint32_t)ipt;
  uint32_t s = 0;
  for (int k = 0; k < ipt; k++) s += (base + k < n) ? ((in[base + k] + pad) & ~pad) : 0u;
  sh[threadIdx.x] = s;
  __syncthreads();
  for (int st = 128; st >= 1; st >>= 1) {
    if ((int)threadIdx.x < st) sh[threadIdx.x] += sh[threadIdx.x + st];
    __syncthreads();
  }
  if (threadIdx.x == 0) bsum[blockIdx.x] = sh[0];
}

__global__ void __launch_bounds__(1024)
k_scan_top(uint32_t* __restrict__ bsum, uint32_t nblk) {
  __shared__ uint32_t sh[1024];
  uint32_t v[4];
  uint32_t s = 0;
#pragma unroll
  for (int k = 0; k < 4; k++) {
    uint32_t idx = threadIdx.x * 4 + k;
    v[k] = idx < nblk ? bsum[idx] : 0u;
    s += v[k];
  }
  sh[threadIdx.x] = s;
  __syncthreads();
  for (int off = 1; off < 1024; off <<= 1) {
    uint32_t t = (int)threadIdx.x >= off ? sh[threadIdx.x - off] : 0u;
    __syncthreads();
    sh[threadIdx.x] += t;
    __syncthreads();
  }
  uint32_t run = sh[threadIdx.x] - s;
#pragma unroll
  for (int k = 0; k < 4; k++) {
    uint32_t idx = threadIdx.x * 4 + k;
    if (idx < nblk) bsum[idx] = run;
    run += v[k];
  }
}

__global__ void __launch_bounds__(256)
k_scan_apply(uint32_t* __restrict__ counts, uint32_t n, int ipt, uint32_t pad, const uint32_t* __restrict__ bsum,
             uint32_t* __restrict__ offsets) {
  __shared__ uint32_t sh[256];
  uint32_t base = (blockIdx.x * 256u + threadIdx.x) * (uint32_t)ipt;
  uint32_t v[kScanMaxIpt];
  uint32_t s = 0;
#pragma unroll
  for (int k = 0; k < kScanMaxIpt; k++) {
    v[k] = (k < ipt && base + k < n) ? ((counts[base + k] + pad) & ~pad) : 0u;
    s += v[k];
  }
  sh[threadIdx.x] = s;
  __syncthreads();
  for (int off = 1; off < 256; off <<= 1) {
    uint32_t t = (int)threadIdx.x >= off ? sh[threadIdx.x - off] : 0u;
    __syncthreads();
    sh[threadIdx.x] += t;
    __syncthreads();
  }
  uint32_t run = bsum[blockIdx.x] + sh[threadIdx.x] - s;
#pragma unroll
  for (int k = 0; k < kScanMaxIpt; k++) {
    if (k < ipt && base + k < n) {
      offsets[base + k] = run;
      counts[base + k] = 0;
      if (base + k + 1 == n) offsets[n] = run + v[k];
    }
    run += v[k];
  }
}

cudaError_t launch_exclusive_scan(uint32_t* counts, uint32_t n, uint32_t* bsum, uint32_t* offsets, cudaStream_t st,
                                  uint32_t pad) {
  if (n == 0) return cudaMemsetAsync(offsets, 0, 4, st);
  int ipt = 4;
  while ((uint64_t)4096 * 256 * ipt < n && ipt < kScanMaxIpt) ipt *= 2;
  uint32_t per = 256u * (uint32_t)ipt;
  uint32_t nblk = (n + per - 1) / per;
  if (nblk > 4096) return cudaErrorInvalidValue;
  k_scan_block_sums<<<nblk, 256, 0, st>>>(counts, n, ipt, pad, bsum);
  k_scan_top<<<1, 1024, 0, st>>>(bsum, nblk);
  k_scan_apply<<<nblk, 256, 0, st>>>(counts, n, ipt, pad, bsum, offsets);
  return cudaGetLastError();
}

__global__ void __launch_bounds__(256)
k_big_mark_large(const uint32_t* __restrict__ offsets, int shift, uint32_t nb, uint32_t large_thresh,
                 uint32_t* __restrict__ meta, BigLargeRec* __restrict__ large, BigSliceRec* __restrict__ slices) {
// ... 303 lines not shown
  for (int i = lo; i < hi; i++) {
    G1Xyzz p = in[(size_t)j * pin + i];
    xyzz_add(acc, acc, p);
  }
  out[t] = acc;
}

__global__ void k_big_horner(const G1Xyzz* __restrict__ S, BigMsmDims dm, int normalize, G1Jac* __restrict__ out) {
  if (threadIdx.x >= 4 || blockIdx.x != 0) return;
  const Quad q;
  G1Xyzz acc;
  xyzz_set_inf(acc);
#pragma unroll 1
  for (int j = dm.nlocal - 1; j >= 0; j--) {
    if (j != dm.nlocal - 1) {
#pragma unroll 1
      for (int k = 0; k < dm.c * dm.wstep; k++) qxyzz_dbl(q, acc, acc);
    }
    const G1Xyzz s = S[j];
    qxyzz_add(q, acc, acc, s);
  }
#pragma unroll 1
  for (int k = 0; k < dm.c * dm.wfirst; k++) qxyzz_dbl(q, acc, acc);
  G1Jac r;
  if (normalize) {
    G1Affine a;
    qxyzz_to_affine(q, a, acc);
    jac_from_affine(r, a);
  } else {
    xyzz_to_jac(r, acc);
  }
  if (q.lane == 0) out[0] = r;
}

__global__ void k_big_combine(const G1Jac* __restrict__ in, int n, G1Jac* __restrict__ out) {
  if (threadIdx.x != 0 || blockIdx.x != 0) return;
  G1Jac acc;
  jac_set_inf(acc);
#pragma unroll 1
  for (int i = 0; i < n; i++) {
    G1Jac p = in[i];
    jac_add(acc, acc, p);
  }
  G1Affine a;
  jac_to_affine(a, acc);
  jac_from_affine(acc, a);
  out[0] = acc;
}

int big_msm_pick_c(size_t n) {
  int lg = 0;
  while (((size_t)1 << (lg + 1)) <= n) lg++;
  static const int table[] = {8, 8, 8, 8, 8, 8, 8, 8, 8, 8, 8, 9, 11, 12, 12, 15, 16, 16, 16, 16, 16};
  return lg <= 20 ? table[lg] : 16;
}

static int big_msm_pick_rounds(size_t mean) {
  static const int forced = [] {
    const char* e = getenv("CDL_MSM_BATCH_AFFINE");
    return e ? atoi(e) : -1;
  }();
  if (forced >= 0) return forced > kBigMaxBaRounds ? kBigMaxBaRounds : forced;
  int lg = 0;
  while (((size_t)2 << lg) <= mean) lg++;
  int r = lg <= 5 ? lg - 3 : lg - 4;
  return r < 0 ? 0 : r > kBigMaxBaRounds ? kBigMaxBaRounds : r;
}

BigMsmDims big_msm_dims(size_t n, int c, int wfirst, int wstep, int ba_rounds) {
  BigMsmDims d;
  d.n = (int)n;
  d.c = c;
  d.W = (128 + c - 1) / c;
  d.M = 1 << (c - 1);
  d.wfirst = wfirst;
  d.wstep = wstep;
  d.nlocal = wfirst < d.W ? (d.W - wfirst + wstep - 1) / wstep : 0;
  d.nb = (uint32_t)d.nlocal * (uint32_t)d.M;
  size_t mean = 2 * n / (size_t)d.M + 1;
  d.R = ba_rounds >= 0 ? (ba_rounds > kBigMaxBaRounds ? kBigMaxBaRounds : ba_rounds) : big_msm_pick_rounds(mean);
  if (d.nlocal == 0 || n == 0) d.R = 0;
  size_t lt = 8 * ((mean >> d.R) + 1);
  d.large = (uint32_t)(lt < 64 ? 64 : lt > kBigLargeBucket ? kBigLargeBucket : lt);
  return d;
}

static inline size_t al256(size_t x) { return (x + 255) & ~(size_t)255; }

constexpr uint32_t kBaTargetPairs = 24;
static uint32_t ba_grid(uint64_t npairs, int sm_count) {
  static const uint32_t per_sm = [] {
    int of = 0, ob = 0;
    cudaOccupancyMaxActiveBlocksPerMultiprocessor(&of, k_ba_fwd<false>, kBaThreads, 0);
    cudaOccupancyMaxActiveBlocksPerMultiprocessor(&ob, k_ba_bwd<false>, kBaThreads, 0);
    if (of < 1) of = 1;
    if (ob < 1) ob = 1;
    uint32_t a = (uint32_t)of, b = (uint32_t)ob, g = a, h = b;
    while (h) { uint32_t t = g % h; g = h; h = t; }
    return a / g * b;
  }();
  const uint64_t wave = (uint64_t)per_sm * (uint64_t)sm_count;
  if (npairs < wave * kBaThreads * 2) return (uint32_t)((npairs + 2 * kBaThreads - 1) / (2 * kBaThreads));
  uint64_t m = (npairs + wave * kBaThreads * kBaTargetPairs / 2) / (wave * kBaThreads * kBaTargetPairs);
  if (m < 1) m = 1;
  return (uint32_t)(m * wave);
}

struct BigLayout {
  size_t counts, offsets, bsum, meta, entries, buckets, large, slices, slice_out, red0, red1, bins, bin_off, order, tab;
  size_t work0, work1, pre, totals, tpre, total;
  uint32_t max_slices, max_large;
};

static BigLayout big_layout(const BigMsmDims& d) {
  BigLayout L;
  size_t nent = (size_t)big_msm_entries(d);
  size_t nfinal = nent >> d.R;
  L.max_large = (uint32_t)(nfinal / d.large + 1);
  L.max_slices = (uint32_t)(nfinal / kBigSliceLen + L.max_large + 1);
  size_t o = 0;
  L.counts = o; o += al256(((size_t)d.nb + 1) * 4);
  L.offsets = o; o += al256(((size_t)d.nb + 2) * 4);
  L.bsum = o; o += al256(4096 * 4);
  L.meta = o; o += 256;
  L.entries = o; o += al256((nent + 2) * 4);
  L.buckets = o; o += al256(((size_t)d.nb + 1) * sizeof(G1Xyzz));
  L.large = o; o += al256((size_t)L.max_large * sizeof(BigLargeRec));
  L.slices = o; o += al256((size_t)L.max_slices * sizeof(BigSliceRec));
  L.slice_out = o; o += al256((size_t)L.max_slices * sizeof(G1Xyzz));
  size_t red = ((size_t)d.nb / 2 + (size_t)d.nlocal + 1) * sizeof(G1Xyzz);
  L.red0 = o; o += al256(red);
  L.red1 = o; o += al256(red);
  L.bins = o; o += al256(((size_t)kBigLargeBucket + 2) * 4);
  L.bin_off = o; o += al256(((size_t)kBigLargeBucket + 3) * 4);
  L.order = o; o += al256(((size_t)d.nb + 1) * 4);
  L.tab = o; o += al256((2 * (size_t)d.n + 1) * sizeof(BigPoint));
  L.work0 = L.work1 = L.pre = L.totals = L.tpre = o;
  if (d.R > 0) {
    size_t p1 = nent / 2 + 1;
    size_t ntot = (p1 / 2 / kBaThreads + 2) * kBaThreads;
    L.work0 = o; o += al256(p1 * sizeof(G1Affine));
    L.work1 = o; o += al256((p1 / 2 + 1) * sizeof(G1Affine));
    L.pre = o; o += al256(p1 * sizeof(Fp));
    L.totals = o; o += al256(ntot * sizeof(Fp));
    L.tpre = o; o += al256(ntot * sizeof(Fp));
  }
  L.total = o;
  return L;
}

size_t big_msm_scratch_bytes(const BigMsmDims& d) { return big_layout(d).total; }

cudaError_t launch_big_msm(const G1Affine* points, const Fr* scalars, const BigMsmDims& d, int normalize,
                           void* scratch, int sm_count, G1Jac* d_out, cudaStream_t st) {
  msm_l2_carveout(false);
  uint8_t* base = (uint8_t*)scratch;
  BigLayout L = big_layout(d);
  uint32_t* counts = (uint32_t*)(base + L.counts);
  uint32_t* offsets = (uint32_t*)(base + L.offsets);
  uint32_t* bsum = (uint32_t*)(base + L.bsum);
  uint32_t* meta = (uint32_t*)(base + L.meta);
  uint32_t* entries = (uint32_t*)(base + L.entries);
  G1Xyzz* buckets = (G1Xyzz*)(base + L.buckets);
  BigLargeRec* large = (BigLargeRec*)(base + L.large);
  BigSliceRec* slices = (BigSliceRec*)(base + L.slices);
  G1Xyzz* slice_out = (G1Xyzz*)(base + L.slice_out);
  G1Xyzz* red[2] = {(G1Xyzz*)(base + L.red0), (G1Xyzz*)(base + L.red1)};
  uint32_t* bins = (uint32_t*)(base + L.bins);
  uint32_t* bin_off = (uint32_t*)(base + L.bin_off);
  uint32_t* order = (uint32_t*)(base + L.order);
  BigPoint* tab = (BigPoint*)(base + L.tab);

  if (d.nlocal == 0 || d.n == 0) {
    G1Xyzz* one = red[0];
    cudaMemsetAsync(one, 0, sizeof(G1Xyzz), st);
    BigMsmDims e = d;
    e.nlocal = 1; e.wfirst = 0; e.wstep = 1; e.c = 0;
    k_big_horner<<<1, 32, 0, st>>>(one, e, normalize, d_out);
    return cudaGetLastError();
  }
  const uint32_t nb = d.nb;
  const int R = d.R;
  const uint64_t nent = big_msm_entries(d);
  cudaMemsetAsync(counts, 0, ((size_t)nb + 1) * 4, st);
  cudaMemsetAsync(meta, 0, 256, st);
  const int gd = (d.n + 255) / 256;
  k_big_tables<<<gd, 256, 0, st>>>(points, d.n, tab);
  k_big_digits<0><<<gd, 256, 0, st>>>(scalars, d.n, d, counts, nullptr, nullptr);
  cudaError_t se = launch_exclusive_scan(counts, nb, bsum, offsets, st, (1u << R) - 1u);
  if (se != cudaSuccess) return se;
  if (R > 0) cudaMemsetAsync(entries, 0xff, (size_t)(nent + 2) * 4, st);
  k_big_digits<1><<<gd, 256, 0, st>>>(scalars, d.n, d, counts, offsets, entries);

  BigSrc src{tab, (uint32_t)d.n, entries, nullptr};
  if (R > 0) {
    G1Affine* work[2] = {(G1Affine*)(base + L.work0), (G1Affine*)(base + L.work1)};
    Fp* pre = (Fp*)(base + L.pre);
    Fp* totals = (Fp*)(base + L.totals);
    Fp* tpre = (Fp*)(base + L.tpre);
    for (int r = 1; r <= R; r++) {
      const uint64_t npairs = nent >> r;
      if (npairs == 0) break;
      const uint32_t nblk = ba_grid(npairs, sm_count);
      const uint32_t ntot = nblk * (uint32_t)kBaThreads;
      constexpr uint32_t kBaInvThreadsPerSm = 256;
      int G = (int)(ntot / ((uint32_t)sm_count * kBaInvThreadsPerSm));
      G = G < 1 ? 1 : G > 256 ? 256 : G;
      G1Affine* dst = work[(r - 1) & 1];
      if (r == 1) k_ba_fwd<false><<<nblk, kBaThreads, 0, st>>>(src, offsets + nb, r - 1, pre, totals);
      else k_ba_fwd<true><<<nblk, kBaThreads, 0, st>>>(src, offsets + nb, r - 1, pre, totals);
      k_ba_inv<<<(ntot + kBaThreads * G - 1) / (kBaThreads * G), kBaThreads, 0, st>>>(totals, tpre, ntot, G);
      if (r == 1) k_ba_bwd<false><<<nblk, kBaThreads, 0, st>>>(src, offsets + nb, r - 1, pre, totals, dst);
      else k_ba_bwd<true><<<nblk, kBaThreads, 0, st>>>(src, offsets + nb, r - 1, pre, totals, dst);
      src.direct = dst;
    }
  }

  k_big_mark_large<<<(nb + 255) / 256, 256, 0, st>>>(offsets, R, nb, d.large, meta, large, slices);
  const uint32_t nbins = d.large + 1;
  cudaMemsetAsync(bins, 0, ((size_t)nbins + 1) * 4, st);
  k_big_size_sort<0><<<(nb + 255) / 256, 256, 0, st>>>(offsets, R, nb, d.large, bins, nullptr, nullptr);
  se = launch_exclusive_scan(bins, nbins, bsum, bin_off, st);
  if (se != cudaSuccess) return se;
  k_big_size_sort<1><<<(nb + 255) / 256, 256, 0, st>>>(offsets, R, nb, d.large, bins, bin_off, order);
  if (src.direct) {
    k_big_accum<true><<<(nb + 127) / 128, 128, 0, st>>>(src, offsets, R, order, nb, d.large, buckets);
    k_big_slice<true><<<sm_count * 4, kBigCtaThreads, 0, st>>>(src, meta, slices, slice_out);
  } else {
    k_big_accum<false><<<(nb + 127) / 128, 128, 0, st>>>(src, offsets, R, order, nb, d.large, buckets);
    k_big_slice<false><<<sm_count * 4, kBigCtaThreads, 0, st>>>(src, meta, slices, slice_out);
  }
  k_big_large_finish<<<sm_count, kBigCtaThreads, 0, st>>>(meta, large, slice_out, buckets);
  int Lc = d.M < 8 ? d.M : 8;
  int per = d.M / Lc;
  int total = d.nlocal * per;
  if (total <= kBigQuadMaxOutputs) k_big_reduce1_quad<<<(4 * total + 127) / 128, 128, 0, st>>>(buckets, d.M, Lc, total, red[0]);
  else k_big_reduce1<<<(total + 127) / 128, 128, 0, st>>>(buckets, d.M, Lc, total, red[0]);
  int cur = 0;
  while (per > 1) {
    int G = per > 256 ? 16 : (per > 16 ? 8 : per);
    int pout = (per + G - 1) / G;
    int tot = d.nlocal * pout;
    if (tot <= kBigQuadMaxOutputs) k_big_sum_quad<<<(4 * tot + 127) / 128, 128, 0, st>>>(red[cur], per, G, pout, tot, red[cur ^ 1]);
    else k_big_sum<<<(tot + 127) / 128, 128, 0, st>>>(red[cur], per, G, pout, tot, red[cur ^ 1]);
    cur ^= 1;
    per = pout;
  }
  k_big_horner<<<1, 32, 0, st>>>(red[cur], d, normalize, d_out);
  return cudaGetLastError();
}

void launch_big_combine(const G1Jac* in, int n, G1Jac* out, cudaStream_t st) {
  k_big_combine<<<1, 32, 0, st>>>(in, n, out);
}

}
```

go-curdleproofs_b200/csrc/launch.h:

```cpp
#pragma once
#include <cuda_runtime.h>
#include <cstddef>
#include <cstdint>
#include "g1.cuh"
#include "fixed_base.cuh"

namespace cdl {

struct MsmTask {
  uint32_t term_off;
  uint32_t term_cnt;
  uint32_t out_idx;
  uint32_t pad;
};
struct ElemOp {
  uint32_t src, add, dst, sc;
};
constexpr uint32_t kNoPoint = 0xffffffffu;
struct CopyRange {
  uint32_t src, dst, count, pad;
};
constexpr size_t kMsmMaxSmem = 220 * 1024;
constexpr size_t kMsmMaxTerms = kMsmMaxSmem / 36;

void launch_compress(const G1Affine* in, uint8_t* out, int n, cudaStream_t s);
void launch_decompress(const uint8_t* in, G1Affine* out, uint8_t* status, int n, cudaStream_t s);
void launch_fp_mul(const Fp* a, const Fp* b, Fp* out, int n, cudaStream_t s);
void launch_peak(int kind, void* out, int blocks, int tpb, int iters, uint32_t seed, cudaStream_t s);
void launch_scalar_mul(const G1Affine* P, const Fr* s, int stride, const G1Affine* L, G1Affine* out, int n,
                       cudaStream_t st);
void launch_jac_to_affine(const G1Jac* in, G1Affine* out, int n, cudaStream_t st);
void launch_elem_ops(G1Affine* pool, const ElemOp* ops, const Fr* scalars, int n, cudaStream_t st,
                     FixedTable ft = FixedTable());
constexpr int kMatchC = 8;
constexpr uint32_t kMatchTile = 256;
void launch_match_prep(Fr* ks, uint32_t V, int32_t* owner, uint32_t T, cudaStream_t st);
void launch_match_shared(const G1Affine* rg, const G1Affine* krg, uint32_t T, const Fr* ks, uint32_t V,
                         int32_t* owner, cudaStream_t st);
void launch_match_windows(const G1Affine* rg, uint32_t nt, G1Jac* out, cudaStream_t st);
void launch_match_table(const G1Affine* tab, const G1Affine* krg, uint32_t t0, uint32_t nt, const Fr* ks,
                        uint32_t V, int32_t* owner, cudaStream_t st);
template <int C = kFbC>
size_t fixed_table_bytes(uint32_t nbase);
template <int C = kFbC>
void launch_fixed_build(const G1Affine* bases, uint32_t nbase, G1Affine* tab, cudaStream_t st);
void launch_copy_ranges(G1Affine* pool, const CopyRange* ranges, int n, cudaStream_t st);
constexpr int kVsMaxM = 16;
struct VsParams {
  Fr a1b, a2c0, a3d0, a4xf, a5xf, a6xf, a7, a8, beta_inv, sH_host;
  Fr gamma[kVsMaxM], gamma_inv[kVsMaxM], ch[kVsMaxM];
  uint32_t sc_base;
  uint32_t as_base;
  uint32_t pad[2];
};
void launch_verify_scalars(const VsParams* params, const Fr* as, Fr* sc, uint32_t nproofs, uint32_t ell, uint32_t n,
                           uint32_t m, cudaStream_t st);
void launch_compress_idx(const G1Affine* pool, const uint32_t* src, uint8_t* out48, int n, cudaStream_t s);
void launch_decompress_idx(const uint8_t* in48, G1Affine* pool, const uint32_t* dst, uint8_t* status, int n,
                           cudaStream_t s);
cudaError_t msm_small_init();
struct MsmSub {
  uint32_t term_off, term_cnt;
};
struct MsmTask2 {
  uint32_t sub_off, sub_cnt, out_idx, pad;
};
constexpr uint32_t kMsmIdxFixed = 1u << 30;
constexpr uint32_t kMsmChunk = 128;
size_t msm_tp_scratch_bytes(size_t nterm, size_t nsub, size_t ntasks);
uint32_t msm_tp_pick_chunk(size_t nterm, int sm_count);
void msm_l2_carveout(bool on);
void launch_msm_tp(const G1Affine* points, const uint32_t* idx, const Fr* scalars, int nterm, const MsmSub* subs,
                   int nsub, const MsmTask2* tasks, int ntasks, G1Affine* out_aff, uint8_t* out_c48, void* scratch,
                   cudaStream_t st, FixedTable ft = FixedTable(), const uint32_t* fixed_subs = nullptr,
                   int nfixed_subs = 0);
template <class VecSub, class VecTask2>
inline void msm_build_subs(const MsmTask* tasks, size_t ntasks, uint32_t chunk, VecSub& subs, VecTask2& tasks2) {
  subs.clear();
  tasks2.clear();
  for (size_t j = 0; j < ntasks; j++) {
    MsmTask2 t2{(uint32_t)subs.size(), 0, tasks[j].out_idx, 0};
    for (uint32_t o = 0; o < tasks[j].term_cnt; o += chunk) {
      uint32_t c = tasks[j].term_cnt - o < chunk ? tasks[j].term_cnt - o : chunk;
      subs.push_back(MsmSub{tasks[j].term_off + o, c});
      t2.sub_cnt++;
    }
    tasks2.push_back(t2);
  }
}

cudaError_t launch_exclusive_scan(uint32_t* counts, uint32_t n, uint32_t* bsum, uint32_t* offsets, cudaStream_t st,
                                  uint32_t pad = 0);

constexpr int kMsmSplitThreshold = 96;
constexpr size_t kMsmSplitTerms = 384;
void launch_msm_small(const G1Affine* points, const uint32_t* idx, const Fr* scalars, const MsmTask* tasks,
                      int ntasks, size_t max_terms, G1Affine* out_aff, uint8_t* out_c48, cudaStream_t st);


struct BigMsmDims {
  int n, c, W, M, wfirst, wstep, nlocal;
  uint32_t nb;
  uint32_t large;
  int R;
};
constexpr size_t kBigMsmThreshold = 1024;
int big_msm_pick_c(size_t n);
BigMsmDims big_msm_dims(size_t n, int c, int wfirst, int wstep, int ba_rounds = -1);
constexpr int kBigMaxBaRounds = 8;
size_t big_msm_scratch_bytes(const BigMsmDims& d);
inline uint64_t big_msm_entries(const BigMsmDims& d) {
  return 2ull * (uint64_t)d.n * (uint64_t)d.nlocal + (uint64_t)d.nb * (((uint64_t)1 << d.R) - 1);
}
cudaError_t launch_big_msm(const G1Affine* points, const Fr* scalars, const BigMsmDims& d, int normalize,
                           void* scratch, int sm_count, G1Jac* d_out, cudaStream_t st);
void launch_big_combine(const G1Jac* in, int n, G1Jac* out, cudaStream_t st);

}
```

include/curdle_b200.h:

```cpp
#ifndef CURDLE_B200_H
#define CURDLE_B200_H

#include <stddef.h>
#include <stdint.h>

#ifdef __cplusplus
extern "C" {
#endif

typedef struct cdl_ctx cdl_ctx;

typedef enum cdl_status {
  CDL_OK = 0,
  CDL_ERR_NO_DEVICE = -1,
  CDL_ERR_CUDA = -2,
  CDL_ERR_INVALID_ARG = -3,
  CDL_ERR_DECODE = -4,
  CDL_ERR_PROTOCOL = -5,
  CDL_ERR_TOO_LARGE = -6,
  CDL_ERR_INTERNAL = -7
} cdl_status;

typedef struct cdl_fp { uint64_t l[6]; } cdl_fp;
typedef struct cdl_fr { uint64_t l[4]; } cdl_fr;
typedef struct cdl_g1_affine { cdl_fp x, y; } cdl_g1_affine;
typedef struct cdl_g1_jac { cdl_fp x, y, z; } cdl_g1_jac;

int32_t cdl_create(int device, cdl_ctx** out);
void cdl_destroy(cdl_ctx* ctx);
const char* cdl_last_error(cdl_ctx* ctx);
uint32_t cdl_abi_version(void);
int32_t cdl_device_info(cdl_ctx* ctx, int32_t* sm_count, int32_t* clock_khz, char* name, size_t name_cap);


int32_t cdl_g1_msm(cdl_ctx* ctx, const cdl_g1_affine* points, const cdl_fr* scalars, size_t n, cdl_g1_jac* out);

int32_t cdl_g1_msm_batch(cdl_ctx* ctx, const cdl_g1_affine* points, const cdl_fr* scalars,
                         const uint32_t* offsets, size_t k, cdl_g1_affine* out);

int32_t cdl_g1_scalar_mul_affine(cdl_ctx* ctx, const cdl_g1_affine* in, const cdl_fr* s, size_t n,
                                 size_t scalar_stride, cdl_g1_affine* out);

int32_t cdl_g1_fold(cdl_ctx* ctx, cdl_g1_affine* L, const cdl_g1_affine* R, const cdl_fr* x, size_t n);

int32_t cdl_g1_batch_to_affine(cdl_ctx* ctx, const cdl_g1_jac* in, size_t n, cdl_g1_affine* out);

int32_t cdl_g1_sum_affine(cdl_ctx* ctx, const cdl_g1_affine* in, size_t n, cdl_g1_affine* out);

int32_t cdl_g1_compress(cdl_ctx* ctx, const cdl_g1_affine* in, size_t n, uint8_t* out48);

int32_t cdl_g1_decompress(cdl_ctx* ctx, const uint8_t* in48, size_t n, cdl_g1_affine* out, uint8_t* status);


typedef struct cdl_rand cdl_rand;
typedef struct cdl_crs cdl_crs;

#define CDL_N_BLINDERS 4
#define CDL_WHISK_SHUFFLE_PROOF_SIZE 4576
#define CDL_WHISK_TRACKER_SIZE 96

int32_t cdl_rand_new(uint64_t seed, cdl_rand** out);
void cdl_rand_free(cdl_rand* r);
int32_t cdl_rand_get_frs(cdl_rand* r, size_t n, cdl_fr* out);
int32_t cdl_rand_get_g1_affines(cdl_ctx* ctx, cdl_rand* r, size_t n, cdl_g1_affine* out);
int32_t cdl_rand_generate_permutation(cdl_rand* r, size_t n, uint32_t* out);

int32_t cdl_crs_generate(cdl_ctx* ctx, size_t ell, cdl_rand* r, cdl_crs** out);
int32_t cdl_crs_from_points(cdl_ctx* ctx, size_t ell, const cdl_g1_affine* points, cdl_crs** out);
int32_t cdl_crs_export(cdl_ctx* ctx, const cdl_crs* crs, cdl_g1_affine* points);
size_t cdl_crs_ell(const cdl_crs* crs);
int32_t cdl_set_fixed_base_min_batch(cdl_ctx* ctx, int32_t instances);
void cdl_crs_free(cdl_crs* crs);

int32_t cdl_shuffle_permute_commit(cdl_ctx* ctx, const cdl_crs* crs, const cdl_g1_affine* Rs, const cdl_g1_affine* Ss,
                                   const uint32_t* perm, const cdl_fr* k, cdl_rand* r, cdl_g1_affine* Ts,
                                   cdl_g1_affine* Us, cdl_g1_jac* M, cdl_fr* rs_m);

int32_t cdl_prove(cdl_ctx* ctx, const cdl_crs* crs, const cdl_g1_affine* Rs, const cdl_g1_affine* Ss,
                  const cdl_g1_affine* Ts, const cdl_g1_affine* Us, const cdl_g1_jac* M, const uint32_t* perm,
                  const cdl_fr* k, const cdl_fr* rs_m, cdl_rand* r, uint8_t* proof, size_t proof_cap,
                  size_t* proof_len);

int32_t cdl_verify(cdl_ctx* ctx, const cdl_crs* crs, const uint8_t* proof, size_t proof_len,
                   const cdl_g1_affine* Rs, const cdl_g1_affine* Ss, const cdl_g1_affine* Ts,
                   const cdl_g1_affine* Us, const cdl_g1_jac* M, cdl_rand* r, int32_t* ok);

int32_t cdl_whisk_generate_shuffle_proof(cdl_ctx* ctx, const cdl_crs* crs, const uint8_t* pre_trackers,
                                         cdl_rand* r, uint8_t* post_trackers, uint8_t* proof, size_t proof_cap);
int32_t cdl_whisk_is_valid_shuffle_proof(cdl_ctx* ctx, const cdl_crs* crs, const uint8_t* pre_trackers,
                                         const uint8_t* post_trackers, size_t n_pre, size_t n_post,
                                         const uint8_t* proof, size_t proof_len, cdl_rand* r, int32_t* ok);

int32_t cdl_whisk_generate_shuffle_proof_batch(cdl_ctx* ctx, const cdl_crs* crs, size_t B,
                                               const uint8_t* pre_trackers, cdl_rand* const* rands,
                                               uint8_t* post_trackers, uint8_t* proofs, size_t proof_cap,
                                               int32_t* status);
int32_t cdl_whisk_is_valid_shuffle_proof_batch(cdl_ctx* ctx, const cdl_crs* crs, size_t B,
                                               const uint8_t* pre_trackers, const uint8_t* post_trackers,
                                               const uint8_t* proofs, size_t proof_len, cdl_rand* const* rands,
                                               int32_t* ok, int32_t* status);
#define CDL_WHISK_TRACKER_PROOF_SIZE 128
int32_t cdl_whisk_generate_tracker_proof_batch(cdl_ctx* ctx, size_t B, const uint8_t* trackers, const cdl_fr* ks,
                                               cdl_rand* const* rands, uint8_t* proofs, int32_t* status);
int32_t cdl_whisk_is_valid_tracker_proof_batch(cdl_ctx* ctx, size_t B, const uint8_t* trackers, const uint8_t* k_comms,
                                               const uint8_t* proofs, int32_t* ok, int32_t* status);
#define CDL_WHISK_MATCH_MAX (1u << 24)
int32_t cdl_whisk_match_trackers(cdl_ctx* ctx, size_t T, const uint8_t* trackers,
                                 size_t V, const cdl_fr* ks, int32_t* owner, int32_t* status);

int32_t cdl_host_selftest(uint8_t* out32, const cdl_fr* a, const cdl_fr* b, cdl_fr* fr_out);
int32_t cdl_host_selftest_fibers(uint32_t n, uint32_t rounds, uint8_t* digest32, int32_t* used_x8);
int32_t cdl_engine_stats(cdl_ctx* ctx, uint64_t* launches, double* ms, double* modmul, double* bytes, int reset);
int32_t cdl_engine_busy_ms(cdl_ctx* ctx, double* busy_ms);
int32_t cdl_set_lanes(cdl_ctx* ctx, int32_t lanes);
uint64_t cdl_launch_count(cdl_ctx* ctx);


int32_t cdl_dev_alloc(cdl_ctx* ctx, size_t bytes, void** d_ptr);
int32_t cdl_dev_free(cdl_ctx* ctx, void* d_ptr);
int32_t cdl_dev_upload(cdl_ctx* ctx, void* d_dst, const void* h_src, size_t bytes);
int32_t cdl_dev_download(cdl_ctx* ctx, void* h_dst, const void* d_src, size_t bytes);

int32_t cdl_g1_scalar_mul_affine_device(cdl_ctx* ctx, const cdl_g1_affine* d_in, const cdl_fr* d_s, size_t n,
                                        size_t scalar_stride, cdl_g1_affine* d_out);

int32_t cdl_g1_fold_device(cdl_ctx* ctx, cdl_g1_affine* d_L, const cdl_g1_affine* d_R, const cdl_fr* d_x, size_t n);

int32_t cdl_g1_msm_batch_device(cdl_ctx* ctx, cdl_g1_affine* d_pool, const uint32_t* idx, const cdl_fr* scalars,
                                const uint32_t* offsets, size_t k, const uint32_t* out_slot, cdl_g1_affine* out,
                                uint8_t* out48);

int32_t cdl_g1_msm_device(cdl_ctx* ctx, const cdl_g1_affine* d_points, const cdl_fr* d_scalars, size_t n,
                          uint32_t part_index, uint32_t part_count, int32_t normalize, cdl_g1_jac* d_out,
                          float* kernel_ms);
int32_t cdl_set_msm_window(cdl_ctx* ctx, int32_t window_bits);
int32_t cdl_set_msm_batch_affine(cdl_ctx* ctx, int32_t rounds);

int32_t cdl_comm_unique_id(uint8_t* id128);
int32_t cdl_comm_init(cdl_ctx* ctx, const uint8_t* id128, int32_t rank, int32_t world);
int32_t cdl_comm_destroy(cdl_ctx* ctx);
void cdl_comm_partition(size_t n, int32_t world, int32_t rank, int32_t window_bits, int32_t* first_window,
                        int32_t* window_step, int32_t* n_windows, int32_t* my_windows);
int32_t cdl_g1_msm_sharded_device(cdl_ctx* ctx, const cdl_g1_affine* d_points, const cdl_fr* d_scalars, size_t n,
                                  cdl_g1_jac* d_out, float* kernel_ms);
int32_t cdl_g1_msm_sharded(cdl_ctx* ctx, const cdl_g1_affine* points, const cdl_fr* scalars, size_t n,
                           cdl_g1_jac* out);

int32_t cdl_fp_mul(cdl_ctx* ctx, const cdl_fp* a, const cdl_fp* b, size_t n, cdl_fp* out);
int32_t cdl_int_peak(cdl_ctx* ctx, int kind, int iters, double* ops_per_s, double* ms);
int32_t cdl_int_peak_cfg(cdl_ctx* ctx, int kind, int iters, int blocks_per_sm, int threads_per_block,
                         double* ops_per_s, double* ms);

#ifdef __cplusplus
}
#endif
#endif
```

integration/gpu/protocol.go:

```go
package gpu

import "C"

import (
	"unsafe"

	bls12381 "github.com/consensys/gnark-crypto/ecc/bls12-381"
	"github.com/consensys/gnark-crypto/ecc/bls12-381/fr"
)

type Rand struct{ h *C.cdl_rand }

func NewRand(seed uint64) (*Rand, error) {
	var h *C.cdl_rand
	if rc := C.cdl_rand_new(C.uint64_t(seed), &h); rc != 0 {
		return nil, errStatus(rc)
	}
	return &Rand{h}, nil
}

func (r *Rand) Free() { C.cdl_rand_free(r.h) }

func (r *Rand) GetFrs(n int) ([]fr.Element, error) {
	out := make([]fr.Element, n)
	if rc := C.cdl_rand_get_frs(r.h, C.size_t(n), frPtr(out)); rc != 0 {
		return nil, errStatus(rc)
	}
	return out, nil
}

type statusError int32

func (e statusError) Error() string { return "curdle_b200 status " + itoa(int(e)) }
func errStatus(rc C.int32_t) error  { return statusError(rc) }
func itoa(v int) string {
	if v == 0 {
		return "0"
	}
	neg := v < 0
	if neg {
		v = -v
	}
	var b [20]byte
	i := len(b)
	for v > 0 {
		i--
		b[i] = byte('0' + v%10)
		v /= 10
	}
	if neg {
		i--
		b[i] = '-'
	}
	return string(b[i:])
}

type CRS struct {
	h   *C.cdl_crs
	Ell int
}

func (c *Context) GenerateCRS(size int, r *Rand) (*CRS, error) {
	var h *C.cdl_crs
	if rc := C.cdl_crs_generate(c.h, C.size_t(size), r.h, &h); rc != 0 {
		return nil, c.err(rc)
	}
	return &CRS{h, size}, nil
}

func (c *Context) CRSFromPoints(ell int, pts []bls12381.G1Affine) (*CRS, error) {
	var h *C.cdl_crs
	if rc := C.cdl_crs_from_points(c.h, C.size_t(ell), affPtr(pts), &h); rc != 0 {
		return nil, c.err(rc)
	}
	return &CRS{h, ell}, nil
}

func (s *CRS) Free() { C.cdl_crs_free(s.h) }

func (c *Context) Prove(crs *CRS, Rs, Ss, Ts, Us []bls12381.G1Affine, M *bls12381.G1Jac, perm []uint32,
	k *fr.Element, rsM []fr.Element, r *Rand) ([]byte, error) {
	buf := make([]byte, 48*(18+10*32)+32*7+40)
	var n C.size_t
	rc := C.cdl_prove(c.h, crs.h, affPtr(Rs), affPtr(Ss), affPtr(Ts), affPtr(Us),
		(*C.cdl_g1_jac)(unsafe.Pointer(M)), (*C.uint32_t)(unsafe.Pointer(&perm[0])),
		(*C.cdl_fr)(unsafe.Pointer(k)), frPtr(rsM), r.h, (*C.uint8_t)(unsafe.Pointer(&buf[0])), C.size_t(len(buf)), &n)
	if rc != 0 {
		return nil, c.err(rc)
	}
	return buf[:n], nil
}

func (c *Context) Verify(crs *CRS, proof []byte, Rs, Ss, Ts, Us []bls12381.G1Affine, M *bls12381.G1Jac, r *Rand) (bool, error) {
	var ok C.int32_t
	rc := C.cdl_verify(c.h, crs.h, (*C.uint8_t)(unsafe.Pointer(&proof[0])), C.size_t(len(proof)),
		affPtr(Rs), affPtr(Ss), affPtr(Ts), affPtr(Us), (*C.cdl_g1_jac)(unsafe.Pointer(M)), r.h, &ok)
	if rc != 0 {
		return false, c.err(rc)
	}
	return ok == 1, nil
}

const (
	TrackerSize      = C.CDL_WHISK_TRACKER_SIZE
	ShuffleProofSize = C.CDL_WHISK_SHUFFLE_PROOF_SIZE
)

func (c *Context) GenerateWhiskShuffleProofs(crs *CRS, pre []byte, rands []*Rand) (post, proofs []byte, status []int32, err error) {
	B := len(rands)
	post = make([]byte, len(pre))
	proofs = make([]byte, B*ShuffleProofSize)
	status = make([]int32, B)
	hs := make([]*C.cdl_rand, B)
	for i, r := range rands {
		hs[i] = r.h
	}
	rc := C.cdl_whisk_generate_shuffle_proof_batch(c.h, crs.h, C.size_t(B), (*C.uint8_t)(unsafe.Pointer(&pre[0])),
		(**C.cdl_rand)(unsafe.Pointer(&hs[0])), (*C.uint8_t)(unsafe.Pointer(&post[0])),
		(*C.uint8_t)(unsafe.Pointer(&proofs[0])), C.size_t(ShuffleProofSize), (*C.int32_t)(unsafe.Pointer(&status[0])))
	if rc != 0 {
		err = c.err(rc)
	}
	return
}

func (c *Context) IsValidWhiskShuffleProofs(crs *CRS, pre, post, proofs []byte, rands []*Rand) (ok, status []int32, err error) {
	B := len(rands)
	ok = make([]int32, B)
	status = make([]int32, B)
	hs := make([]*C.cdl_rand, B)
	for i, r := range rands {
		hs[i] = r.h
	}
	rc := C.cdl_whisk_is_valid_shuffle_proof_batch(c.h, crs.h, C.size_t(B), (*C.uint8_t)(unsafe.Pointer(&pre[0])),
		(*C.uint8_t)(unsafe.Pointer(&post[0])), (*C.uint8_t)(unsafe.Pointer(&proofs[0])), C.size_t(ShuffleProofSize),
		(**C.cdl_rand)(unsafe.Pointer(&hs[0])), (*C.int32_t)(unsafe.Pointer(&ok[0])), (*C.int32_t)(unsafe.Pointer(&status[0])))
	if rc != 0 {
		err = c.err(rc)
	}
	return
}

func (c *Context) MatchWhiskTrackers(trackers []byte, ks []fr.Element) (owner, status []int32, err error) {
	if len(trackers) == 0 || len(trackers)%TrackerSize != 0 || len(ks) == 0 {
		return nil, nil, errStatus(C.int32_t(C.CDL_ERR_INVALID_ARG))
	}
	T := len(trackers) / TrackerSize
	owner = make([]int32, T)
	status = make([]int32, T)
	rc := C.cdl_whisk_match_trackers(c.h, C.size_t(T), (*C.uint8_t)(unsafe.Pointer(&trackers[0])), C.size_t(len(ks)),
		frPtr(ks), (*C.int32_t)(unsafe.Pointer(&owner[0])), (*C.int32_t)(unsafe.Pointer(&status[0])))
	if rc != 0 {
		return nil, nil, c.err(rc)
	}
	return owner, status, nil
}
```

Before: 5264.

## Add randomized batch verification that folds all proof MSMs into one

When at least a threshold of proofs is verified together (default 64), each per-proof MSM task is weighted by a random scalar. The weights come from a hash of the transcripts and the verifier's own random coefficients. All weighted terms, with repeated CRS bases merged, go into a single large MSM. If the result is the point at infinity, every proof is accepted and the per-task MSMs are skipped; otherwise the code falls back to per-proof checking. This removes many small MSMs for large batches, at the cost of an extra large MSM that is wasted when any proof fails, and extra host hashing.

Result: faster. 5805, median of 6 (+10.3%).

```diff
diff --git a/go-curdleproofs_b200/binding.py b/go-curdleproofs_b200/binding.py
--- a/go-curdleproofs_b200/binding.py
+++ b/go-curdleproofs_b200/binding.py
@@ -105,6 +105,7 @@
     lib.cdl_set_msm_window.argtypes = [vp, i32]
     lib.cdl_set_msm_batch_affine.argtypes = [vp, i32]
     lib.cdl_set_fixed_base_min_batch.argtypes = [vp, i32]
+    lib.cdl_set_batch_verify_min.argtypes = [vp, i32]
     lib.cdl_comm_unique_id.argtypes = [vp]
     lib.cdl_comm_init.argtypes = [vp, vp, i32, i32]
     lib.cdl_comm_destroy.argtypes = [vp]
@@ -314,6 +315,10 @@
     self._chk(self.lib.cdl_set_fixed_base_min_batch(self.h, instances))
 
 
+def _ctx_set_batch_verify_min(self, proofs: int):
+    self._chk(self.lib.cdl_set_batch_verify_min(self.h, proofs))
+
+
 def _ctx_set_msm_batch_affine(self, rounds: int):
     self._chk(self.lib.cdl_set_msm_batch_affine(self.h, rounds))
 
@@ -549,6 +554,7 @@
 Context.set_msm_window = _ctx_set_msm_window
 Context.set_msm_batch_affine = _ctx_set_msm_batch_affine
 Context.set_fixed_base_min_batch = _ctx_set_fixed_base_min_batch
+Context.set_batch_verify_min = _ctx_set_batch_verify_min
 Context.comm_init = _ctx_comm_init
 Context.comm_destroy = _ctx_comm_destroy
 Context.g1_msm_sharded_device = _ctx_g1_msm_sharded_device
diff --git a/go-curdleproofs_b200/csrc/capi.cu b/go-curdleproofs_b200/csrc/capi.cu
--- a/go-curdleproofs_b200/csrc/capi.cu
+++ b/go-curdleproofs_b200/csrc/capi.cu
@@ -29,7 +29,7 @@
 
 extern "C" {
 
-uint32_t cdl_abi_version(void) { return (1u << 16) | 5u; }
+uint32_t cdl_abi_version(void) { return (1u << 16) | 6u; }
 
 int32_t cdl_create(int device, cdl_ctx** out) {
   if (!out) return CDL_ERR_INVALID_ARG;
diff --git a/go-curdleproofs_b200/csrc/capi_protocol.cu b/go-curdleproofs_b200/csrc/capi_protocol.cu
--- a/go-curdleproofs_b200/csrc/capi_protocol.cu
+++ b/go-curdleproofs_b200/csrc/capi_protocol.cu
@@ -318,6 +318,13 @@
   if (!c || instances < -1) return CDL_ERR_INVALID_ARG;
   std::lock_guard<std::mutex> lk(c->mu);
   c->root()->fixed_min_batch = instances;
+  return CDL_OK;
+}
+
+int32_t cdl_set_batch_verify_min(cdl_ctx* c, int32_t proofs) {
+  if (!c || proofs < -1) return CDL_ERR_INVALID_ARG;
+  std::lock_guard<std::mutex> lk(c->mu);
+  c->root()->batch_verify_min = proofs;
   return CDL_OK;
 }
 
diff --git a/go-curdleproofs_b200/csrc/context.cuh b/go-curdleproofs_b200/csrc/context.cuh
--- a/go-curdleproofs_b200/csrc/context.cuh
+++ b/go-curdleproofs_b200/csrc/context.cuh
@@ -32,6 +32,7 @@
   int comm_rank = 0, comm_world = 1;
   int msm_c_override = 0;
   int fixed_min_batch = -1;
+  int batch_verify_min = -1;
   int msm_ba_override = -1;
   cdl_ctx* parent = nullptr;
   std::vector<cdl_ctx*> lanes;
diff --git a/go-curdleproofs_b200/csrc/engine.cu b/go-curdleproofs_b200/csrc/engine.cu
--- a/go-curdleproofs_b200/csrc/engine.cu
+++ b/go-curdleproofs_b200/csrc/engine.cu
@@ -64,7 +64,8 @@
   if (d_pool_) cudaFree(d_pool_);
   if (d_win_) cudaFree(d_win_);
   if (d_match_) cudaFree(d_match_);
-  for (Staging* s : {&s_idx_, &s_sc_, &s_task_, &s_out_, &s_ops_, &s_enc_, &s_st_, &s_jac_, &s_sub_, &s_t2_, &s_cr_, &s_vs_, &s_as_, &s_fsub_}) {
+  if (d_bv_) cudaFree(d_bv_);
+  for (Staging* s : {&s_idx_, &s_sc_, &s_task_, &s_out_, &s_ops_, &s_enc_, &s_st_, &s_jac_, &s_sub_, &s_t2_, &s_cr_, &s_vs_, &s_as_, &s_fsub_, &s_bv_}) {
     if (s->h) cudaFreeHost(s->h);
     if (s->d) cudaFree(s->d);
   }
@@ -272,8 +273,7 @@
 
 static constexpr uint32_t kFixedMinTerms = 16;
 
-int32_t Engine::run_msm(MsmStage& st, const std::function<int32_t(cdl::Fr* d_scalars)>& before,
-                        const G1Affine* points) {
+int32_t Engine::run_msm(MsmStage& st, const MsmBefore& before, const G1Affine* points) {
   ProfScope ps(prof.gpu);
   size_t nt = st.tasks.size(), nterm = st.idx.size();
   st.out48.resize(nt * 48);
@@ -310,8 +310,13 @@
   CDL_CUDA(ctx_, cudaMemcpyAsync(s_sc_.d, s_sc_.h, nterm * 32, cudaMemcpyHostToDevice, ctx_->stream));
   CDL_CUDA(ctx_, cudaMemcpyAsync(s_task_.d, s_task_.h, nt * sizeof(MsmTask), cudaMemcpyHostToDevice, ctx_->stream));
   if (before) {
-    int32_t brc = before((cdl::Fr*)s_sc_.d);
+    bool done = false;
+    int32_t brc = before((const uint32_t*)s_idx_.d, (cdl::Fr*)s_sc_.d, (const MsmTask*)s_task_.d, done);
     if (brc) return brc;
+    if (done) {
+      std::fill(st.out48.begin(), st.out48.end(), 0);
+      return CDL_OK;
+    }
   }
   double alg = 0;
   for (size_t j = 0; j < st.tasks.size(); j++)
diff --git a/go-curdleproofs_b200/csrc/engine_verify.cu b/go-curdleproofs_b200/csrc/engine_verify.cu
--- a/go-curdleproofs_b200/csrc/engine_verify.cu
+++ b/go-curdleproofs_b200/csrc/engine_verify.cu
@@ -11,6 +11,8 @@
 namespace {
 
 const uint8_t kInfEncV[48] = {0xc0};
+
+constexpr uint32_t kBatchVerifyMinDefault = 64;
 
 struct VState {
   Transcript tr{"curdleproofs"};
@@ -22,6 +24,8 @@
   Fr sp_alpha, sp_beta, p, gp_alpha, gp_beta, gp_beta_inv, z;
   Rand snapshot{0};
   bool have_snapshot = false;
+  Fr aw[8] = {};
+  uint8_t digest[32] = {};
   void fail(const std::string& e) { if (!failed) { failed = true; err = e; } }
 };
 
@@ -46,6 +50,68 @@
   }
 };
 
+inline size_t al256(size_t x) { return (x + 255) & ~(size_t)255; }
+
+}
+
+int32_t Engine::batch_check(const MsmStage& st, const std::vector<Fr>& rho, uint32_t crs_size, const uint32_t* d_idx,
+                            const cdl::Fr* d_sc, const MsmTask* d_tasks, bool* all_inf) {
+  *all_inf = false;
+  const uint32_t nterm = (uint32_t)st.idx.size(), nt = (uint32_t)st.tasks.size();
+  const size_t nc = (size_t)nterm + crs_size;
+  const cdl::BigMsmDims d = cdl::big_msm_dims(nc, cdl::big_msm_pick_c(nc), 0, 1);
+  if (!nterm || nc >= ((size_t)1 << 30) || cdl::big_msm_entries(d) >= ((uint64_t)1 << 32)) return CDL_OK;
+  std::vector<uint32_t> off(crs_size + 1, 0);
+  for (uint32_t j = 0; j < nterm; j++)
+    if (st.idx[j] < crs_size) off[st.idx[j] + 1]++;
+  for (uint32_t b = 0; b < crs_size; b++) off[b + 1] += off[b];
+  const uint32_t npos = off[crs_size];
+  const size_t h_off = al256((size_t)nt * 32), h_pos = h_off + al256(((size_t)crs_size + 1) * 4),
+               h_flag = h_pos + al256((size_t)npos * 4);
+  int32_t rc;
+  if ((rc = reserve(s_bv_, h_flag + 4))) return rc;
+  uint8_t* hb = (uint8_t*)s_bv_.h;
+  memcpy(hb, rho.data(), (size_t)nt * 32);
+  memcpy(hb + h_off, off.data(), off.size() * 4);
+  uint32_t* pos = (uint32_t*)(hb + h_pos);
+  for (uint32_t j = 0; j < nterm; j++)
+    if (st.idx[j] < crs_size) pos[off[st.idx[j]]++] = j;
+  const size_t d_csc = al256(nc * 4), d_res = d_csc + al256(nc * 32), d_flag = d_res + al256(sizeof(cdl::G1Jac)),
+               d_scr = d_flag + 256, need = d_scr + cdl::big_msm_scratch_bytes(d);
+  if (need > bv_cap_) {
+    cudaStreamSynchronize(ctx_->stream);
+    if (d_bv_) cudaFree(d_bv_);
+    d_bv_ = nullptr;
+    bv_cap_ = 0;
+    if (cudaMalloc(&d_bv_, need + need / 4) != cudaSuccess) {
+      cudaGetLastError();
+      return CDL_OK;
+    }
+    bv_cap_ = need + need / 4;
+  }
+  uint8_t* db = (uint8_t*)d_bv_;
+  const uint8_t* sb = (const uint8_t*)s_bv_.d;
+  uint32_t* cidx = (uint32_t*)db;
+  cdl::Fr* csc = (cdl::Fr*)(db + d_csc);
+  cdl::G1Jac* res = (cdl::G1Jac*)(db + d_res);
+  uint32_t* flag = (uint32_t*)(db + d_flag);
+  CDL_CUDA(ctx_, cudaMemcpyAsync(s_bv_.d, s_bv_.h, h_flag, cudaMemcpyHostToDevice, ctx_->stream));
+  tick();
+  cdl::launch_bv_assemble(d_idx, d_sc, d_tasks, nt, (const cdl::Fr*)sb, nterm, (const uint32_t*)(sb + h_off),
+                          (const uint32_t*)(sb + h_pos), crs_size, cidx, csc, ctx_->stream);
+  int nk = 0;
+  cudaError_t e = cdl::launch_big_msm(d_pool_, csc, d, 0, db + d_scr, ctx_->sm_count, res, ctx_->stream, cidx,
+                                      false, &nk);
+  cdl::launch_bv_is_inf(res, flag, ctx_->stream);
+  tock(0, msm_algorithmic_modmul(nc), 128.0 * nc);
+  launches += 2 + nk;
+  CDL_CUDA(ctx_, e);
+  CDL_CUDA(ctx_, cudaGetLastError());
+  CDL_CUDA(ctx_, cudaMemcpyAsync(hb + h_flag, flag, 4, cudaMemcpyDeviceToHost, ctx_->stream));
+  CDL_CUDA(ctx_, ctx_->sync_stream());
+  finish_timing();
+  *all_inf = *(const uint32_t*)(hb + h_flag) == 1;
+  return CDL_OK;
 }
 
 int32_t Engine::verify(const Layout& L, uint32_t B, const cdl_crs* crs, std::vector<ParsedProof>& pp,
@@ -136,6 +202,9 @@
   const bool dev_sc = device_scalars && L.m <= (uint32_t)cdl::kVsMaxM;
   std::vector<cdl::VsParams> vsp(dev_sc ? B : 0);
   std::vector<uint32_t> merged_at(B, 0);
+  const int32_t bv_set = ctx_->root()->batch_verify_min;
+  const uint32_t bv_min = bv_set >= 0 ? (uint32_t)bv_set : kBatchVerifyMinDefault;
+  const bool bv_maybe = bv_min > 0 && B >= bv_min;
   par(B, [&](size_t b) {
     VState& s = *S[b];
     if (s.failed) return;
@@ -150,7 +219,7 @@
     std::vector<Fr>& sc = t_sc[b];
     auto neg_term = [&](uint32_t point, const Fr& coeff) { idx.push_back(point); sc.push_back(fr_neg(coeff)); };
 
-    Fr a1 = rand.get_fr();
+    Fr a1 = s.aw[0] = rand.get_fr();
     const Fr a1b = fr_mul(a1, s.sp_beta);
     if (!dev_sc)
       for (uint32_t i = 0; i < ell; i++) sGs[i] = a1b;
@@ -196,7 +265,7 @@
           svp[i + (1u << j)] = fr_mul(svp[i], gamma_inv[m - j - 1]);
         }
     }
-    Fr a2 = rand.get_fr();
+    Fr a2 = s.aw[1] = rand.get_fr();
     const Fr a2c0 = fr_mul(a2, c0);
     if (!dev_sc) {
       for (uint32_t i = 0; i < ell; i++) sGs[i] = fr_add(sGs[i], fr_mul(a2c0, sv[i]));
@@ -210,7 +279,7 @@
     neg_term(q.pt[w.B_c], a2);
     neg_term(q.pt[w.C], fr_mul(a2, ipa_alpha));
     sH = fr_sub(sH, fr_mul(a2, fr_mul(fr_mul(fr_mul(ipa_alpha, ipa_alpha), s.z), ipa_beta)));
-    Fr a3 = rand.get_fr();
+    Fr a3 = s.aw[2] = rand.get_fr();
     const Fr a3d0 = fr_mul(a3, d0);
     if (!dev_sc) {
       for (uint32_t i = 0; i < ell; i++) sGs[i] = fr_add(sGs[i], fr_mul(a3d0, fr_mul(svp[i], us[i])));
@@ -282,7 +351,7 @@
         for (uint32_t j = 0; j < lg_n; j++)
           for (uint32_t i = 0; i < (1u << j); i++) xs[i + (1u << j)] = fr_mul(xs[i], ch[lg_n - 1 - j]);
       }
-      Fr a4 = rand.get_fr();
+      Fr a4 = s.aw[3] = rand.get_fr();
       if (!dev_sc) {
         for (uint32_t i = 0; i < ell; i++) sGs[i] = fr_add(sGs[i], fr_mul(a4, xs[i]));
         sHs[0] = fr_add(sHs[0], fr_mul(a4, xs[ell]));
@@ -296,7 +365,7 @@
         neg_term(q.pt[w.L_A + i], fr_mul(a4, ch[i]));
         neg_term(q.pt[w.R_A + i], fr_mul(a4, ch_inv[i]));
       }
-      Fr a5 = rand.get_fr();
+      Fr a5 = s.aw[4] = rand.get_fr();
       if (!dev_sc) {
         for (uint32_t i = 0; i < ell; i++) sTs[i] = fr_add(sTs[i], fr_mul(a5, xs[i]));
         sH = fr_add(sH, fr_mul(a5, xs[ell + 2]));
@@ -307,7 +376,7 @@
         neg_term(q.pt[w.L_T + i], fr_mul(a5, ch[i]));
         neg_term(q.pt[w.R_T + i], fr_mul(a5, ch_inv[i]));
       }
-      Fr a6 = rand.get_fr();
+      Fr a6 = s.aw[5] = rand.get_fr();
       if (!dev_sc) {
         for (uint32_t i = 0; i < ell; i++) sUs[i] = fr_add(sUs[i], fr_mul(a6, xs[i]));
         sH = fr_add(sH, fr_mul(a6, xs[ell + 3]));
@@ -318,11 +387,11 @@
         neg_term(q.pt[w.L_U + i], fr_mul(a6, ch[i]));
         neg_term(q.pt[w.R_U + i], fr_mul(a6, ch_inv[i]));
       }
-      Fr a7 = rand.get_fr();
+      Fr a7 = s.aw[6] = rand.get_fr();
       if (!dev_sc)
         for (uint32_t i = 0; i < ell; i++) sRs[i] = fr_mul(a7, s.as[i]);
       neg_term(q.pt[w.R], a7);
-      Fr a8 = rand.get_fr();
+      Fr a8 = s.aw[7] = rand.get_fr();
       if (!dev_sc)
         for (uint32_t i = 0; i < ell; i++) sSs[i] = fr_mul(a8, s.as[i]);
       neg_term(q.pt[w.S], a8);
@@ -359,6 +428,15 @@
     }
     idx.swap(all_idx);
     sc.swap(all_sc);
+    if (bv_maybe) {
+      Transcript t = s.tr;
+      uint8_t c[32];
+      t.challenge_bytes("batch_verify_weights", c, 32);
+      Shake256 h;
+      h.absorb(c, 32);
+      h.absorb(reinterpret_cast<const uint8_t*>(s.aw), sizeof s.aw);
+      h.read(s.digest, 32);
+    }
   });
 
   st.clear();
@@ -384,8 +462,8 @@
       k++;
     }
   }
-  if (dev_sc && !vs_launch.empty()) {
-    const size_t np = vs_launch.size();
+  const size_t np = vs_launch.size();
+  if (np) {
     if ((rc = reserve(s_vs_, np * sizeof(cdl::VsParams))) || (rc = reserve(s_as_, (size_t)B * ell * 32))) return rc;
     memcpy(s_vs_.h, vs_launch.data(), np * sizeof(cdl::VsParams));
     Fr* as_h = (Fr*)s_as_.h;
@@ -394,22 +472,44 @@
     });
     CDL_CUDA(ctx_, cudaMemcpyAsync(s_vs_.d, s_vs_.h, np * sizeof(cdl::VsParams), cudaMemcpyHostToDevice, ctx_->stream));
     CDL_CUDA(ctx_, cudaMemcpyAsync(s_as_.d, s_as_.h, (size_t)B * ell * 32, cudaMemcpyHostToDevice, ctx_->stream));
-    rc = run_msm(st, [&](cdl::Fr* d_sc) -> int32_t {
+  }
+  uint32_t nin = 0;
+  for (uint32_t b = 0; b < B; b++) nin += first_task[b] >= 0;
+  const bool combined = bv_maybe && nin >= bv_min;
+  std::vector<Fr> rho;
+  if (combined) {
+    static const char kLabel[] = "curdleproofs_b200 batch verify";
+    Shake256 h;
+    h.absorb(reinterpret_cast<const uint8_t*>(kLabel), sizeof kLabel - 1);
+    for (uint32_t b = 0; b < B; b++)
+      if (first_task[b] >= 0) h.absorb(S[b]->digest, 32);
+    rho.resize(st.tasks.size());
+    for (Fr& r : rho) {
+      uint64_t w[4] = {0, 0, 0, 0};
+      h.read(reinterpret_cast<uint8_t*>(w), 16);
+      if (!w[0] && !w[1]) w[0] = 1;
+      r = fr_from_canonical(w);
+    }
+  }
+  bool all_pass = false;
+  rc = run_msm(st, [&](const uint32_t* d_idx, cdl::Fr* d_sc, const MsmTask* d_tasks, bool& done) -> int32_t {
+    if (np) {
       cdl::launch_verify_scalars((const cdl::VsParams*)s_vs_.d, (const cdl::Fr*)s_as_.d, d_sc, (uint32_t)np, ell, n, L.m,
                                  ctx_->stream);
       launches++;
-      return CDL_OK;
-    });
-  } else {
-    rc = run_msm(st);
-  }
+    }
+    if (!combined) return CDL_OK;
+    int32_t r = batch_check(st, rho, L.crs_size, d_idx, d_sc, d_tasks, &all_pass);
+    done = all_pass;
+    return r;
+  });
   if (rc) return rc;
   for (uint32_t b = 0; b < B; b++) {
     VState& s = *S[b];
     if (s.failed) { status[b] = CDL_ERR_PROTOCOL; errs[b] = s.err; continue; }
     const uint8_t* o = st.out48.data() + 48 * (size_t)first_task[b];
     bool same_scalar_ok = true;
-    for (int t = 0; t < 4; t++) same_scalar_ok = same_scalar_ok && memcmp(o + 48 * t, kInfEncV, 48) == 0;
+    for (int t = 0; t < 4 && !all_pass; t++) same_scalar_ok = same_scalar_ok && memcmp(o + 48 * t, kInfEncV, 48) == 0;
     if (!same_scalar_ok) {
       verdict[b] = 0;
       if (s.have_snapshot) rands[b]->r = s.snapshot;
@@ -421,7 +521,7 @@
       if (s.have_snapshot) rands[b]->r = s.snapshot;
       continue;
     }
-    verdict[b] = memcmp(o + 48 * 4, kInfEncV, 48) == 0 ? 1 : 0;
+    verdict[b] = all_pass || memcmp(o + 48 * 4, kInfEncV, 48) == 0 ? 1 : 0;
   }
   return CDL_OK;
 }
diff --git a/go-curdleproofs_b200/csrc/host/engine.hpp b/go-curdleproofs_b200/csrc/host/engine.hpp
--- a/go-curdleproofs_b200/csrc/host/engine.hpp
+++ b/go-curdleproofs_b200/csrc/host/engine.hpp
@@ -112,8 +112,8 @@
   int32_t copy_ranges(const std::vector<cdl::CopyRange>& ranges);
   int32_t compress(const std::vector<uint32_t>& src, std::vector<uint8_t>& out48);
   int32_t decompress(const uint8_t* enc48, const std::vector<uint32_t>& dst, std::vector<uint8_t>& status);
-  int32_t run_msm(MsmStage& st, const std::function<int32_t(cdl::Fr* d_scalars)>& before = nullptr,
-                  const cdl::G1Affine* points = nullptr);
+  using MsmBefore = std::function<int32_t(const uint32_t* d_idx, cdl::Fr* d_scalars, const cdl::MsmTask* d_tasks, bool& done)>;
+  int32_t run_msm(MsmStage& st, const MsmBefore& before = nullptr, const cdl::G1Affine* points = nullptr);
   int32_t run_elem(const std::vector<cdl::ElemOp>& ops, const std::vector<Fr>& sc);
   int32_t match_trackers(uint32_t T, const Fr* ks, uint32_t V, int32_t* owner);
 
@@ -163,12 +163,16 @@
   void* d_match_ = nullptr;
   size_t match_cap_ = 0;
   bool match_scratch(uint32_t tile);
+  void* d_bv_ = nullptr;
+  size_t bv_cap_ = 0;
+  int32_t batch_check(const MsmStage& st, const std::vector<Fr>& rho, uint32_t crs_size, const uint32_t* d_idx,
+                      const cdl::Fr* d_sc, const cdl::MsmTask* d_tasks, bool* all_inf);
   struct Staging {
     void* h = nullptr;
     void* d = nullptr;
     size_t cap = 0;
   };
-  Staging s_idx_, s_sc_, s_task_, s_out_, s_ops_, s_enc_, s_st_, s_jac_, s_sub_, s_t2_, s_cr_, s_fsub_, s_vs_, s_as_;
+  Staging s_idx_, s_sc_, s_task_, s_out_, s_ops_, s_enc_, s_st_, s_jac_, s_sub_, s_t2_, s_cr_, s_fsub_, s_vs_, s_as_, s_bv_;
   int32_t reserve(Staging& s, size_t bytes);
   void tick();
   void tock(int cls, double modmul, double bytes);
diff --git a/go-curdleproofs_b200/csrc/k_batch_verify.cu b/go-curdleproofs_b200/csrc/k_batch_verify.cu
--- /dev/null
+++ b/go-curdleproofs_b200/csrc/k_batch_verify.cu
@@ -0,0 +1,55 @@
+#include <cuda_runtime.h>
+#include "fields.cuh"
+#include "launch.h"
+
+namespace cdl {
+
+__global__ void __launch_bounds__(256)
+k_bv_weigh(const uint32_t* __restrict__ idx, const Fr* __restrict__ sc, const MsmTask* __restrict__ tasks, uint32_t ntask,
+           const Fr* __restrict__ rho, uint32_t nterm, uint32_t* __restrict__ cidx, Fr* __restrict__ csc) {
+  const uint32_t j = blockIdx.x * blockDim.x + threadIdx.x;
+  if (j >= nterm) return;
+  uint32_t lo = 0, hi = ntask;
+  while (hi - lo > 1) {
+    const uint32_t mid = (lo + hi) >> 1;
+    if (tasks[mid].term_off <= j) lo = mid;
+    else hi = mid;
+  }
+  Fr s = sc[j];
+  FrM::mul(s, s, rho[lo]);
+  csc[j] = s;
+  cidx[j] = idx[j] & (kMsmIdxFixed - 1u);
+}
+
+__global__ void __launch_bounds__(128)
+k_bv_crs(const uint32_t* __restrict__ off, const uint32_t* __restrict__ pos, uint32_t ncrs, uint32_t nterm,
+         uint32_t* __restrict__ cidx, Fr* __restrict__ csc) {
+  const uint32_t b = blockIdx.x * blockDim.x + threadIdx.x;
+  if (b >= ncrs) return;
+  Fr acc, zero;
+  FrM::set_zero(acc);
+  FrM::set_zero(zero);
+#pragma unroll 1
+  for (uint32_t k = off[b]; k < off[b + 1]; k++) {
+    const uint32_t p = pos[k];
+    FrM::add(acc, acc, csc[p]);
+    csc[p] = zero;
+  }
+  cidx[nterm + b] = b;
+  csc[nterm + b] = acc;
+}
+
+__global__ void k_bv_is_inf(const G1Jac* __restrict__ r, uint32_t* __restrict__ flag) {
+  if (threadIdx.x == 0 && blockIdx.x == 0) flag[0] = jac_is_inf(r[0]) ? 1u : 0u;
+}
+
+void launch_bv_assemble(const uint32_t* idx, const Fr* sc, const MsmTask* tasks, uint32_t ntask, const Fr* rho,
+                        uint32_t nterm, const uint32_t* crs_off, const uint32_t* crs_pos, uint32_t ncrs, uint32_t* cidx,
+                        Fr* csc, cudaStream_t st) {
+  k_bv_weigh<<<(nterm + 255) / 256, 256, 0, st>>>(idx, sc, tasks, ntask, rho, nterm, cidx, csc);
+  k_bv_crs<<<(ncrs + 127) / 128, 128, 0, st>>>(crs_off, crs_pos, ncrs, nterm, cidx, csc);
+}
+
+void launch_bv_is_inf(const G1Jac* r, uint32_t* flag, cudaStream_t st) { k_bv_is_inf<<<1, 32, 0, st>>>(r, flag); }
+
+}
diff --git a/go-curdleproofs_b200/csrc/k_msm_big.cu b/go-curdleproofs_b200/csrc/k_msm_big.cu
--- a/go-curdleproofs_b200/csrc/k_msm_big.cu
+++ b/go-curdleproofs_b200/csrc/k_msm_big.cu
@@ -64,10 +64,10 @@
 }
 
 __global__ void __launch_bounds__(256)
-k_big_tables(const G1Affine* __restrict__ points, int n, BigPoint* __restrict__ tab) {
+k_big_tables(const G1Affine* __restrict__ points, const uint32_t* __restrict__ idx, int n, BigPoint* __restrict__ tab) {
   int i = blockIdx.x * blockDim.x + threadIdx.x;
   if (i >= n) return;
-  const G1Affine p = points[i];
+  const G1Affine p = points[idx ? idx[i] : (uint32_t)i];
   Fp beta, bx;
   fp_set_beta(beta);
   FpM::mul(bx, p.x, beta);
@@ -677,8 +677,9 @@
 size_t big_msm_scratch_bytes(const BigMsmDims& d) { return big_layout(d).total; }
 
 cudaError_t launch_big_msm(const G1Affine* points, const Fr* scalars, const BigMsmDims& d, int normalize,
-                           void* scratch, int sm_count, G1Jac* d_out, cudaStream_t st) {
-  msm_l2_carveout(false);
+                           void* scratch, int sm_count, G1Jac* d_out, cudaStream_t st, const uint32_t* idx,
+                           bool release_l2, int* nkernels) {
+  if (release_l2) msm_l2_carveout(false);
   uint8_t* base = (uint8_t*)scratch;
   BigLayout L = big_layout(d);
   uint32_t* counts = (uint32_t*)(base + L.counts);
@@ -702,6 +703,7 @@
     BigMsmDims e = d;
     e.nlocal = 1; e.wfirst = 0; e.wstep = 1; e.c = 0;
     k_big_horner<<<1, 32, 0, st>>>(one, e, normalize, d_out);
+    if (nkernels) *nkernels = 1;
     return cudaGetLastError();
   }
   const uint32_t nb = d.nb;
@@ -710,7 +712,7 @@
   cudaMemsetAsync(counts, 0, ((size_t)nb + 1) * 4, st);
   cudaMemsetAsync(meta, 0, 256, st);
   const int gd = (d.n + 255) / 256;
-  k_big_tables<<<gd, 256, 0, st>>>(points, d.n, tab);
+  k_big_tables<<<gd, 256, 0, st>>>(points, idx, d.n, tab);
   k_big_digits<0><<<gd, 256, 0, st>>>(scalars, d.n, d, counts, nullptr, nullptr);
   cudaError_t se = launch_exclusive_scan(counts, nb, bsum, offsets, st, (1u << R) - 1u);
   if (se != cudaSuccess) return se;
@@ -761,8 +763,9 @@
   int total = d.nlocal * per;
   if (total <= kBigQuadMaxOutputs) k_big_reduce1_quad<<<(4 * total + 127) / 128, 128, 0, st>>>(buckets, d.M, Lc, total, red[0]);
   else k_big_reduce1<<<(total + 127) / 128, 128, 0, st>>>(buckets, d.M, Lc, total, red[0]);
-  int cur = 0;
+  int cur = 0, nsum = 0;
   while (per > 1) {
+    nsum++;
     int G = per > 256 ? 16 : (per > 16 ? 8 : per);
     int pout = (per + G - 1) / G;
     int tot = d.nlocal * pout;
@@ -772,6 +775,7 @@
     per = pout;
   }
   k_big_horner<<<1, 32, 0, st>>>(red[cur], d, normalize, d_out);
+  if (nkernels) *nkernels = 17 + 3 * R + nsum;
   return cudaGetLastError();
 }
 
diff --git a/go-curdleproofs_b200/csrc/launch.h b/go-curdleproofs_b200/csrc/launch.h
--- a/go-curdleproofs_b200/csrc/launch.h
+++ b/go-curdleproofs_b200/csrc/launch.h
@@ -55,6 +55,10 @@
 };
 void launch_verify_scalars(const VsParams* params, const Fr* as, Fr* sc, uint32_t nproofs, uint32_t ell, uint32_t n,
                            uint32_t m, cudaStream_t st);
+void launch_bv_assemble(const uint32_t* idx, const Fr* sc, const MsmTask* tasks, uint32_t ntask, const Fr* rho,
+                        uint32_t nterm, const uint32_t* crs_off, const uint32_t* crs_pos, uint32_t ncrs, uint32_t* cidx,
+                        Fr* csc, cudaStream_t st);
+void launch_bv_is_inf(const G1Jac* r, uint32_t* flag, cudaStream_t st);
 void launch_compress_idx(const G1Affine* pool, const uint32_t* src, uint8_t* out48, int n, cudaStream_t s);
 void launch_decompress_idx(const uint8_t* in48, G1Affine* pool, const uint32_t* dst, uint8_t* status, int n,
                            cudaStream_t s);
@@ -113,7 +117,8 @@
   return 2ull * (uint64_t)d.n * (uint64_t)d.nlocal + (uint64_t)d.nb * (((uint64_t)1 << d.R) - 1);
 }
 cudaError_t launch_big_msm(const G1Affine* points, const Fr* scalars, const BigMsmDims& d, int normalize,
-                           void* scratch, int sm_count, G1Jac* d_out, cudaStream_t st);
+                           void* scratch, int sm_count, G1Jac* d_out, cudaStream_t st, const uint32_t* idx = nullptr,
+                           bool release_l2 = true, int* nkernels = nullptr);
 void launch_big_combine(const G1Jac* in, int n, G1Jac* out, cudaStream_t st);
 
 }
diff --git a/include/curdle_b200.h b/include/curdle_b200.h
--- a/include/curdle_b200.h
+++ b/include/curdle_b200.h
@@ -70,6 +70,7 @@
 int32_t cdl_crs_export(cdl_ctx* ctx, const cdl_crs* crs, cdl_g1_affine* points);
 size_t cdl_crs_ell(const cdl_crs* crs);
 int32_t cdl_set_fixed_base_min_batch(cdl_ctx* ctx, int32_t instances);
+int32_t cdl_set_batch_verify_min(cdl_ctx* ctx, int32_t proofs);
 void cdl_crs_free(cdl_crs* crs);
 
 int32_t cdl_shuffle_permute_commit(cdl_ctx* ctx, const cdl_crs* crs, const cdl_g1_affine* Rs, const cdl_g1_affine* Ss,
diff --git a/integration/gpu/protocol.go b/integration/gpu/protocol.go
--- a/integration/gpu/protocol.go
+++ b/integration/gpu/protocol.go
@@ -91,6 +91,13 @@
 	return buf[:n], nil
 }
 
+func (c *Context) SetBatchVerifyMin(proofs int) error {
+	if rc := C.cdl_set_batch_verify_min(c.h, C.int32_t(proofs)); rc != 0 {
+		return c.err(rc)
+	}
+	return nil
+}
+
 func (c *Context) Verify(crs *CRS, proof []byte, Rs, Ss, Ts, Us []bls12381.G1Affine, M *bls12381.G1Jac, r *Rand) (bool, error) {
 	var ok C.int32_t
 	rc := C.cdl_verify(c.h, crs.h, (*C.uint8_t)(unsafe.Pointer(&proof[0])), C.size_t(len(proof)),
```
